# r4dl/StopThePop-Rasterization

Hardware: AMD Instinct MI355X
Metric: fwd+bwd frames/sec at 1920×1080, 1M Gaussians; PSNR vs reference (higher is better)
Workload: dtype f32

## Files before the change

### stopthepop-rasterization_amd/csrc/stp_binning.hip

```cpp
#include <cstdlib>
#include <cstring>
#include <rocprim/rocprim.hpp>

#include "stp_internal.h"
#include "stp_device.h"

namespace stp {

uint32_t higher_msb(uint32_t n)
{
    uint32_t msb = sizeof(n) * 4, step = msb;
    while (step > 1) {
        step /= 2;
        if (n >> msb) msb += step; else msb -= step;
    }
    if (n >> msb) msb++;
    return msb;
}

size_t scan_temp_bytes(size_t P)
{
    size_t bytes = 0;
    (void)rocprim::inclusive_scan(nullptr, bytes, (uint32_t*)nullptr, (uint32_t*)nullptr, P, rocprim::plus<uint32_t>());
    return bytes;
}

#include <rocprim/rocprim_version.hpp>
#if ROCPRIM_VERSION_MAJOR == 4 && ROCPRIM_VERSION_MINOR == 2
#define STP_OWN_ONESWEEP 1
#else
#define STP_OWN_ONESWEEP 0
#warning "stp_binning.hip: the own onesweep driver is written against rocPRIM 4.2; with this rocPRIM the tile-bit sort uses rocprim::radix_sort_pairs (check rocprim::detail::onesweep_* against this version, then extend the #if)"
#endif
namespace {
#if STP_OWN_ONESWEEP
namespace rpd = rocprim::detail;
using OsConfig = rpd::wrapped_radix_sort_onesweep_config<rocprim::default_config, uint64_t, uint32_t>;
constexpr rpd::radix_sort_onesweep_config_params os_params()
{
    rpd::radix_sort_onesweep_config_params p = OsConfig::architecture_config<rpd::target_arch::gfx950>::params;
    p.sort.items_per_thread = 8;
#ifdef STP_OS_SORT_BLOCK
    p.sort.block_size = STP_OS_SORT_BLOCK;
#endif
#ifdef STP_OS_SORT_IPT
    p.sort.items_per_thread = STP_OS_SORT_IPT;
#endif
#ifdef STP_OS_HIST_BLOCK
    p.histogram.block_size = STP_OS_HIST_BLOCK;
#endif
#ifdef STP_OS_HIST_IPT
    p.histogram.items_per_thread = STP_OS_HIST_IPT;
#endif
    return p;
}
constexpr rpd::radix_sort_onesweep_config_params OS = os_params();
constexpr unsigned OS_RADIX = 1u << OS.radix_bits_per_place;
constexpr unsigned OS_HIST_ITEMS = OS.histogram.block_size * OS.histogram.items_per_thread;
constexpr unsigned OS_SORT_ITEMS = OS.sort.block_size * OS.sort.items_per_thread;
constexpr unsigned OS_MAX_PLACES = 4;
using OsBlockId = rpd::block_id_wrapper<unsigned int, true>;

struct OsLayout {
    uint32_t* offsets;
    unsigned int* block_ids;
    rpd::onesweep_lookback_state* lookback;
    uint32_t* offsets_tmp;
    uint64_t* keys_tmp;
    uint32_t* values_tmp;
    size_t zero_bytes, total, lookback_offset;
    uint32_t sort_blocks;
};
OsLayout os_layout(char* base, size_t R)
{
    OsLayout L{};
    auto up = [](size_t v) { return (v + 255) & ~(size_t)255; };
    L.sort_blocks = (uint32_t)((R + OS_SORT_ITEMS - 1) / OS_SORT_ITEMS);
    size_t off = 0;
    L.offsets = reinterpret_cast<uint32_t*>(base + off); off += up(sizeof(uint32_t) * OS_MAX_PLACES * OS_RADIX);
    L.block_ids = reinterpret_cast<unsigned int*>(base + off); off += up(sizeof(unsigned int) * OS_MAX_PLACES);
    L.lookback = reinterpret_cast<rpd::onesweep_lookback_state*>(base + off);
    L.lookback_offset = off;
    off += up(sizeof(rpd::onesweep_lookback_state) * OS_MAX_PLACES * OS_RADIX * (size_t)L.sort_blocks);
    L.zero_bytes = off;
    L.offsets_tmp = reinterpret_cast<uint32_t*>(base + off); off += up(sizeof(uint32_t) * OS_RADIX);
    L.keys_tmp = reinterpret_cast<uint64_t*>(base + off); off += up(sizeof(uint64_t) * R);
    L.values_tmp = reinterpret_cast<uint32_t*>(base + off); off += up(sizeof(uint32_t) * R);
    L.total = off;
    return L;
}

__global__ void __launch_bounds__(OS.histogram.block_size) os_histograms_kernel(const uint64_t* keys, uint32_t* counts, uint32_t size, uint32_t full_blocks, unsigned begin_bit, unsigned end_bit)
{
    rpd::onesweep_histograms<OS.histogram.block_size, OS.histogram.items_per_thread, OS.radix_bits_per_place, false>(
        keys, counts, size, full_blocks, rocprim::identity_decomposer{}, begin_bit, end_bit);
}
__global__ void __launch_bounds__(OS.histogram.block_size) os_scan_histograms_kernel(uint32_t* offsets)
{
    rpd::onesweep_scan_histograms<OS.histogram.block_size, OS.radix_bits_per_place>(offsets);
}
__global__ void __launch_bounds__(OS.sort.block_size) os_iteration_kernel(const uint64_t* keys_in, uint64_t* keys_out, const uint32_t* values_in, uint32_t* values_out, unsigned size,
                                                                         uint32_t* offsets_in, uint32_t* offsets_out, rpd::onesweep_lookback_state* lookback, unsigned bit,
                                                                         unsigned radix_bits, unsigned full_blocks, OsBlockId ordered_bid)
{
    rpd::onesweep_iteration<OS.sort.block_size, OS.sort.items_per_thread, OS.radix_bits_per_place, false, OS.radix_rank_algorithm>(
        keys_in, keys_out, values_in, values_out, size, offsets_in, offsets_out, lookback, rocprim::identity_decomposer{}, bit, radix_bits, full_blocks, ordered_bid);
}

constexpr uint32_t OWN_MIN = 1u << 16, OWN_MAX = 1u << 30;
bool own_onesweep_driver(size_t R)
{
    const bool lib = switches().tile_sort == Switches::TILE_SORT_ROCPRIM;
    const bool always = switches().tile_sort == Switches::TILE_SORT_OWN;
    return !lib && (R >= OWN_MIN || (always && R > 0)) && R < OWN_MAX;
}
#else
struct OsLayout { size_t total; };
OsLayout os_layout(char*, size_t) { return OsLayout{0}; }
bool own_onesweep_driver(size_t) { return false; }
#endif
}

size_t sort_temp_bytes(size_t R)
{
    size_t bytes = 0;
    (void)rocprim::radix_sort_pairs(nullptr, bytes, (uint64_t*)nullptr, (uint64_t*)nullptr, (uint32_t*)nullptr, (uint32_t*)nullptr,
                                    R, 0u, 64u);
    const size_t own = os_layout(nullptr, R).total;
    return bytes > own ? bytes : own;
}

void sort_zero_region(const BinningState& b, size_t R, uint32_t tiles, uint32_t** ptr, size_t* words)
{
    *ptr = nullptr; *words = 0;
    if (!own_onesweep_driver(R)) return;
#if STP_OWN_ONESWEEP
    const OsLayout L = os_layout(b.sort_temp, R);
    const uint32_t bit = higher_msb(tiles);
    const size_t places = (bit + OS.radix_bits_per_place - 1) / OS.radix_bits_per_place;
    const size_t bytes = L.lookback_offset + ((sizeof(rpd::onesweep_lookback_state) * places * OS_RADIX * (size_t)L.sort_blocks + 255) & ~(size_t)255);
    *ptr = reinterpret_cast<uint32_t*>(b.sort_temp);
    *words = (bytes < L.zero_bytes ? bytes : L.zero_bytes) / sizeof(uint32_t);
#else
    (void)b; (void)tiles;
#endif
}

hipError_t launch_scan(const FrameParams& f, const GeometryState& g, hipStream_t st)
{
    size_t bytes = g.scan_temp_bytes;
    return rocprim::inclusive_scan(g.scan_temp, bytes, g.tiles_touched, g.point_offsets, (size_t)f.P, rocprim::plus<uint32_t>(), st);
}

hipError_t launch_sort(const FrameParams& f, const BinningState& b, int R, bool tile_bits_only, bool zeroed, hipStream_t st)
{
    if (R <= 0) return hipSuccess;
    const uint32_t bit = higher_msb((uint32_t)(f.gx * f.gy));
    if (!(tile_bits_only && zeroed && own_onesweep_driver((size_t)R))) {
        size_t bytes = b.sort_temp_bytes;
        return rocprim::radix_sort_pairs(b.sort_temp, bytes, b.keys_unsorted, b.keys, b.point_list_unsorted, b.point_list, (size_t)R,
                                         tile_bits_only ? 32u : 0u, 32u + bit, st);
    }
#if STP_OWN_ONESWEEP
    const OsLayout L = os_layout(b.sort_temp, (size_t)R);
    const unsigned begin_bit = 32u, end_bit = 32u + bit;
    const unsigned places = (bit + OS.radix_bits_per_place - 1) / OS.radix_bits_per_place;
    const uint32_t size = (uint32_t)R;
    {
        const uint32_t blocks = (size + OS_HIST_ITEMS - 1) / OS_HIST_ITEMS, full_blocks = size % OS_HIST_ITEMS == 0 ? blocks : blocks - 1;
        hipLaunchKernelGGL(os_histograms_kernel, dim3(blocks), dim3(OS.histogram.block_size), 0, st, b.keys_unsorted, L.offsets, size, full_blocks, begin_bit, end_bit);
        hipLaunchKernelGGL(os_scan_histograms_kernel, dim3(places), dim3(OS.histogram.block_size), 0, st, L.offsets);
    }
    const uint32_t blocks = L.sort_blocks, full_blocks = size % OS_SORT_ITEMS == 0 ? blocks : blocks - 1;
    bool to_output = (places - 1) % 2 == 0, from_input = true;
    for (unsigned place = 0, pbit = begin_bit; place < places; place++, pbit += OS.radix_bits_per_place) {
        const uint64_t* kin = from_input ? b.keys_unsorted : (to_output ? L.keys_tmp : b.keys);
        const uint32_t* vin = from_input ? b.point_list_unsorted : (to_output ? L.values_tmp : b.point_list);
        uint64_t* kout = to_output ? b.keys : L.keys_tmp;
        uint32_t* vout = to_output ? b.point_list : L.values_tmp;
        const unsigned radix_bits = end_bit - pbit < OS.radix_bits_per_place ? end_bit - pbit : OS.radix_bits_per_place;
        hipLaunchKernelGGL(os_iteration_kernel, dim3(blocks), dim3(OS.sort.block_size), 0, st, kin, kout, vin, vout, size, L.offsets + place * OS_RADIX, L.offsets_tmp,
                           L.lookback + (size_t)place * OS_RADIX * blocks, pbit, radix_bits, full_blocks, OsBlockId::create(L.block_ids + place));
        from_input = false;
        to_output = !to_output;
    }
#endif
    return hipGetLastError();
}

namespace {

constexpr int SCAN_THREADS = 1024;

__global__ void __launch_bounds__(SCAN_THREADS) tile_scan_kernel(int tile0, int T, const uint32_t* __restrict__ counts_, uint2* __restrict__ ranges_,
                                                                 uint32_t* __restrict__ cursor_, uint32_t* __restrict__ total)
{
    const uint32_t* __restrict__ counts = counts_ + tile0;
    uint2* __restrict__ ranges = ranges_ + tile0;
    uint32_t* __restrict__ cursor = cursor_ + tile0;
    __shared__ uint32_t s_part[SCAN_THREADS];
    const int tid = (int)threadIdx.x;
    const int per = (T + SCAN_THREADS - 1) / SCAN_THREADS;
    const int lo = min(tid * per, T), hi = min(lo + per, T);
    uint32_t sum = 0;
    for (int t = lo; t < hi; t++) sum += counts[t];
    s_part[tid] = sum;
    __syncthreads();
    for (int off = 1; off < SCAN_THREADS; off <<= 1) {
        const uint32_t v = tid >= off ? s_part[tid - off] : 0u;
        __syncthreads();
        s_part[tid] += v;
        __syncthreads();
    }
    uint32_t run = s_part[tid] - sum;
    for (int t = lo; t < hi; t++) {
        const uint32_t c = counts[t];
        ranges[t] = c ? make_uint2(run, run + c) : make_uint2(0u, 0u);
        cursor[t] = run;
        run += c;
    }
    if (tid == SCAN_THREADS - 1) total[0] = s_part[tid];
}

__global__ void __launch_bounds__(256) bin_pad_kernel(int R, const uint32_t* __restrict__ total, uint64_t* __restrict__ keys, uint32_t* __restrict__ list)
{
    for (int i = (int)total[0] + (int)threadIdx.x; i < R; i += 256) {
        keys[i] = make_sort_key(INVALID_TILE_ID, FLT_MAX);
        list[i] = 0xFFFFFFFFu;
    }
}

}

hipError_t launch_tile_scan(const FrameParams& f, const ImageState& img, hipStream_t st)
{
    hipLaunchKernelGGL(tile_scan_kernel, dim3(1), dim3(SCAN_THREADS), 0, st, f.gx * f.ty0, f.gx * (f.ty1 - f.ty0), img.tile_counts, img.ranges, img.tile_cursor, img.bin_total);
    return hipGetLastError();
}

hipError_t launch_bin_pad(const BinningState& b, const ImageState& img, int R, hipStream_t st)
{
    if (R <= 0) return hipSuccess;
    hipLaunchKernelGGL(bin_pad_kernel, dim3(1), dim3(256), 0, st, R, img.bin_total, b.keys, b.point_list);
    return hipGetLastError();
}

}
```

### stopthepop-rasterization_amd/csrc/stp_buffers.hip

```cpp
#include "stp_internal.h"
#include "stp_layout_cache.h"

#include <cstring>
#include <mutex>
#include <string>

namespace stp {

GeometryState carve_geometry(char* base, size_t P, bool with_inv, size_t* total, NamedOffset* names, int* n_names, float** sh_stash)
{
    Carver c(base);
    GeometryState g{};
    size_t off;
    int n = 0;
    auto note = [&](const char* nm, size_t o, size_t cnt) { if (names) names[n] = {nm, o, cnt}; n++; };
    g.status = c.take<uint32_t>(64, &off);
    g.depths = c.take<float>(P, &off); note("depths", off, P);
    g.clamped = c.take<uint8_t>(3 * P, &off); note("clamped", off, 3 * P);
    g.internal_radii = c.take<int32_t>(P, &off); note("radii", off, P);
    g.rects2D = c.take<float2>(P, &off); note("rects2D", off, 2 * P);
    g.means2D = c.take<float2>(P, &off); note("means2D", off, 2 * P);
    g.cov3D = c.take<float>(6 * P, &off); note("cov3D", off, 6 * P);
    if (with_inv) { g.cov3D_inv = c.take<float4>(3 * P, &off); note("cov3D_inv", off, 12 * P); }
    if (with_inv) { g.gpack = c.take<float4>(4 * P, &off); note("gpack", off, 16 * P); }
    g.conic_opacity = c.take<float4>(P, &off); note("conic_opacity", off, 4 * P);
    g.rgb = c.take<float>(3 * P, &off); note("rgb", off, 3 * P);
    g.tiles_touched = c.take<uint32_t>(P, &off); note("tiles_touched", off, P);
    g.point_offsets = c.take<uint32_t>(P, &off); note("point_offsets", off, P);
    g.block_sums = c.take<uint32_t>((P + 255) / 256, &off);
    g.block_prefix = c.take<uint32_t>((P + 255) / 256, &off);
    g.scan_temp_bytes = scan_temp_bytes(P);
    g.scan_temp = c.take<char>(g.scan_temp_bytes);
    g.invz = c.take<float>(P, &off); note("invz", off, P);
    {
        const Carver before_stash = c;
        float* const stash = c.take<float>(9 * P, &off); note("sh_stash", off, 9 * P);
        if (sh_stash) *sh_stash = stash;
        else c = before_stash;
    }
    if (total) *total = c.total();
    if (n_names) *n_names = n;
    return g;
}

ImageState carve_image(char* base, int W, int H, int ty0, int ty1, int log_depth, size_t* total, NamedOffset* names, int* n_names)
{
    Carver c(base);
    ImageState s{};
    size_t off;
    int n = 0;
    auto note = [&](const char* nm, size_t o, size_t cnt) { if (names) names[n] = {nm, o, cnt}; n++; };
    const int gx = (W + TILE - 1) / TILE;
    const int py0 = ty0 * TILE < H ? ty0 * TILE : H, py1 = ty1 * TILE < H ? ty1 * TILE : H;
    const size_t N = (size_t)W * (size_t)(py1 > py0 ? py1 - py0 : 0), T = (size_t)gx * (size_t)(ty1 > ty0 ? ty1 - ty0 : 0);
    s.header = c.take<uint32_t>(64, &off); note("header", off, 4);
    s.final_T = c.take<float>(N, &off); note("final_T", off, N);
    s.n_contrib = c.take<uint32_t>(N, &off); note("n_contrib", off, N);
    s.ranges = c.take<uint2>(T, &off); note("ranges", off, 2 * T);
    s.dbg_minmax = c.take<uint32_t>(2, &off); note("dbg_minmax", off, 2);
    s.tile_counts = c.take<uint32_t>(T, &off); note("tile_counts", off, T);
    s.tile_cursor = c.take<uint32_t>(T, &off); note("tile_cursor", off, T);
    s.bin_total = c.take<uint32_t>(2, &off); note("bin_total", off, 2);
    s.tile_flags = c.take<uint32_t>(T, &off); note("tile_flags", off, T);
    const size_t recs_per_tile = 4 * (size_t)blend_log_rows(log_depth) * 64;
    s.log_depth = log_depth;
    if (log_depth > 0) {
        const size_t recs = T * recs_per_tile;
        s.blend_log = c.take<uint32_t>(recs / 2, &off); note("blend_log", off, recs);
    }
    if (total) *total = c.total();
    if (n_names) *n_names = n;
    if (base) {
        const size_t pix0 = (size_t)W * (size_t)py0, tile0 = (size_t)gx * (size_t)ty0;
        s.final_T -= pix0; s.n_contrib -= pix0;
        s.ranges -= tile0; s.tile_counts -= tile0; s.tile_cursor -= tile0; s.tile_flags -= tile0;
        if (s.blend_log) s.blend_log -= tile0 * (recs_per_tile / 2);
    }
    return s;
}

BinningState carve_binning(char* base, size_t R, size_t* total, NamedOffset* names, int* n_names)
{
    Carver c(base);
    BinningState b{};
    size_t off;
    int n = 0;
    auto note = [&](const char* nm, size_t o, size_t cnt) { if (names) names[n] = {nm, o, cnt}; n++; };
    b.header = c.take<uint32_t>(64, &off); note("header", off, 4);
    b.point_list = c.take<uint32_t>(R, &off); note("point_list", off, R);
    b.point_list_unsorted = c.take<uint32_t>(R, &off); note("point_list_unsorted", off, R);
    b.keys = c.take<uint64_t>(R, &off); note("keys", off, R);
    b.keys_unsorted = c.take<uint64_t>(R, &off); note("keys_unsorted", off, R);
    b.sort_temp_bytes = sort_temp_bytes(R);
    b.sort_temp = c.take<char>(b.sort_temp_bytes);
    b.entA = c.take<float4>(R, &off); note("entA", off, 4 * R);
    b.entB = c.take<float4>(R, &off); note("entB", off, 4 * R);
    b.entC = c.take<float4>(R, &off); note("entC", off, 4 * R);
    b.entD = c.take<float4>(R, &off); note("entD", off, 4 * R);
    b.entF = c.take<float4>(R, &off); note("entF", off, 4 * R);
    if (total) *total = c.total();
    if (n_names) *n_names = n;
    return b;
}

void clamp_tile_rows(int height, int& y0, int& y1)
{
    const int gy = (height + TILE - 1) / TILE;
    if (y1 <= 0) { y0 = 0; y1 = gy; return; }
    y0 = y0 < 0 ? 0 : (y0 > gy ? gy : y0);
    y1 = y1 > gy ? gy : y1;
    if (y1 < y0) y1 = y0;
}

static std::mutex g_layout_mutex;
static LayoutCache g_layout, g_log_depth, g_stash;
void remember_layout(const void* binning, uint32_t count, int64_t R) { std::lock_guard<std::mutex> l(g_layout_mutex); g_layout.put(binning, count, R); }
void remember_log_depth(const void* image, uint32_t depth, int64_t R) { std::lock_guard<std::mutex> l(g_layout_mutex); g_log_depth.put(image, depth, R); }
void remember_stash(const void* geometry, bool stash, int64_t R) { std::lock_guard<std::mutex> l(g_layout_mutex); g_stash.put(geometry, stash ? 1u : 0u, R); }
static int read_buffer_header(const uint32_t* dev_header, uint32_t magic, const char* what, uint32_t* value, hipStream_t st, bool have_stream)
{
    uint32_t h[4] = {0, 0, 0, 0};
    if (!have_stream) (void)hipDeviceSynchronize();
    if (hipMemcpyAsync(h, dev_header, sizeof(h), hipMemcpyDeviceToHost, have_stream ? st : nullptr) != hipSuccess ||
        hipStreamSynchronize(have_stream ? st : nullptr) != hipSuccess) { (void)hipGetLastError(); return fail(STP_ERR_HIP, std::string("could not read the header of the ") + what + " buffer"); }
    if (h[0] != magic || h[2] != ~h[1])
        return fail(STP_ERR_INVALID_ARGUMENT, std::string("the ") + what + " buffer does not carry a header of this library: it was not written by stp_forward (or has been overwritten)");
    *value = h[1];
    return 0;
}
int layout_of(const char* binning, uint32_t R, uint32_t* cap, hipStream_t st, bool have_stream)
{
    {
        std::lock_guard<std::mutex> l(g_layout_mutex);
        if (g_layout.get(binning, (int64_t)R, cap) && *cap >= R) return 0;
    }
    if (int rc = read_buffer_header(reinterpret_cast<const uint32_t*>(binning), STP_HEADER_MAGIC_BINNING, "binning", cap, st, have_stream)) return rc;
    if (*cap < R) return fail(STP_ERR_INVALID_ARGUMENT, "the binning buffer was carved for fewer entries than num_rendered");
    remember_layout(binning, *cap, (int64_t)R);
    return 0;
}

int log_depth_of(const char* image, int64_t R, uint32_t* depth, hipStream_t st, bool have_stream)
{
    {
        std::lock_guard<std::mutex> l(g_layout_mutex);
        if (g_log_depth.get(image, R, depth)) return 0;
    }
    if (int rc = read_buffer_header(reinterpret_cast<const uint32_t*>(image), STP_HEADER_MAGIC_IMAGE, "image", depth, st, have_stream)) return rc;
    if (*depth != 0u && (int)*depth != blend_log_clamp_depth((int)*depth)) return fail(STP_ERR_INVALID_ARGUMENT, "the image buffer's header holds an impossible blend-log depth");
    remember_log_depth(image, *depth, R);
    return 0;
}

int stash_of(const char* geometry, int P, int64_t R, bool* stash, hipStream_t st, bool have_stream)
{
    uint32_t v = 0;
    {
        std::lock_guard<std::mutex> l(g_layout_mutex);
        if (g_stash.get(geometry, R, &v)) { *stash = v != 0u; return 0; }
    }
    uint32_t h[4] = {0, 0, 0, 0};
    if (!have_stream) (void)hipDeviceSynchronize();
    if (hipMemcpyAsync(h, reinterpret_cast<const uint32_t*>(geometry) + STP_STASH_WORD, sizeof(h), hipMemcpyDeviceToHost, have_stream ? st : nullptr) != hipSuccess ||
        hipStreamSynchronize(have_stream ? st : nullptr) != hipSuccess) { (void)hipGetLastError(); return fail(STP_ERR_HIP, "could not read the status block of the geometry buffer"); }
    *stash = h[0] == STP_HEADER_MAGIC_STASH && h[1] == (uint32_t)P && h[2] == ~(uint32_t)P;
    remember_stash(geometry, *stash, R);
    return 0;
}

}

using namespace stp;

extern "C" {

size_t stp_geometry_buffer_size(int P, const StpSettings* settings)
{
    size_t total = 0;
    carve_geometry(nullptr, (size_t)P, settings ? requires_depth_along_ray(*settings) : true, &total);
    return total;
}
size_t stp_geometry_buffer_size_stash(int P, const StpSettings* settings)
{
    size_t total = 0;
    float* stash = nullptr;
    carve_geometry(nullptr, (size_t)P, settings ? requires_depth_along_ray(*settings) : true, &total, nullptr, nullptr, &stash);
    return total;
}
size_t stp_binning_buffer_size(int R)
{
    size_t total = 0;
    carve_binning(nullptr, (size_t)(R > 0 ? R : 0), &total);
    return total;
}
size_t stp_image_buffer_size(int width, int height)
{
    size_t total = 0;
    carve_image(nullptr, width, height, 0, (height + TILE - 1) / TILE, 0, &total);
    return total;
}

static size_t blend_log_bytes_of(int width, int height, int tile_y0, int tile_y1, int depth)
{
    clamp_tile_rows(height, tile_y0, tile_y1);
    size_t plain = 0, with_log = 0;
    carve_image(nullptr, width, height, tile_y0, tile_y1, 0, &plain);
    carve_image(nullptr, width, height, tile_y0, tile_y1, depth, &with_log);
    return with_log - plain;
}
size_t stp_blend_log_bytes_rows(int width, int height, int tile_y0, int tile_y1)
{
    return blend_log_bytes_of(width, height, tile_y0, tile_y1, blend_log_default_depth());
}
size_t stp_blend_log_bytes(int width, int height) { return stp_blend_log_bytes_rows(width, height, 0, 0); }
size_t stp_blend_log_bytes_depth(int width, int height, int tile_y0, int tile_y1, int depth)
{
    return blend_log_bytes_of(width, height, tile_y0, tile_y1, depth > 0 ? blend_log_clamp_depth(depth) : blend_log_clamp_depth(1 << 30));
}

static int find_name(const NamedOffset* names, int n, const char* name, size_t* offset, size_t* count)
{
    for (int i = 0; i < n; i++)
        if (std::strcmp(names[i].name, name) == 0) {
            if (offset) *offset = names[i].offset;
            if (count) *count = names[i].count;
            return 0;
        }
    return fail(STP_ERR_INVALID_ARGUMENT, std::string("unknown sub-array name: ") + name);
}
int stp_geometry_layout(int P, const StpSettings* settings, const char* name, size_t* offset, size_t* count)
{
    NamedOffset names[24]; int n = 0;
    carve_geometry(nullptr, (size_t)P, settings ? requires_depth_along_ray(*settings) : true, nullptr, names, &n);
    return find_name(names, n, name, offset, count);
}
int stp_binning_layout(int R, const char* name, size_t* offset, size_t* count)
{
    NamedOffset names[16]; int n = 0;
    carve_binning(nullptr, (size_t)(R > 0 ? R : 0), nullptr, names, &n);
    return find_name(names, n, name, offset, count);
}
void stp_forget_buffer(const void* buffer)
{
    if (!buffer) return;
    std::lock_guard<std::mutex> l(g_layout_mutex);
    g_layout.map.erase(buffer);
    g_log_depth.map.erase(buffer);
    g_stash.map.erase(buffer);
}
int stp_blend_log_depth(const void* image_buffer)
{
    if (!image_buffer) return fail(STP_ERR_INVALID_ARGUMENT, "null image buffer");
    uint32_t d = 0;
    if (int rc = log_depth_of((const char*)image_buffer, -1, &d)) return rc;
    return (int)d;
}
int stp_binning_layout_count(const void* binning_buffer, int R)
{
    if (!binning_buffer) return fail(STP_ERR_INVALID_ARGUMENT, "null binning buffer");
    uint32_t cap = 0;
    if (int rc = layout_of((const char*)binning_buffer, (uint32_t)(R > 0 ? R : 0), &cap)) return rc;
    return (int)cap;
}
static int image_layout_of(int width, int height, int tile_y0, int tile_y1, int depth, const char* name, size_t* offset, size_t* count)
{
    NamedOffset names[16]; int n = 0;
    clamp_tile_rows(height, tile_y0, tile_y1);
    carve_image(nullptr, width, height, tile_y0, tile_y1, depth, nullptr, names, &n);
    return find_name(names, n, name, offset, count);
}
int stp_image_layout_rows(int width, int height, int tile_y0, int tile_y1, const char* name, size_t* offset, size_t* count)
{
    return image_layout_of(width, height, tile_y0, tile_y1, blend_log_default_depth(), name, offset, count);
}
int stp_image_layout(int width, int height, const char* name, size_t* offset, size_t* count)
{
    return stp_image_layout_rows(width, height, 0, 0, name, offset, count);
}
int stp_image_layout_depth(int width, int height, int tile_y0, int tile_y1, int log_depth, const char* name, size_t* offset, size_t* count)
{
    return image_layout_of(width, height, tile_y0, tile_y1, log_depth > 0 ? blend_log_clamp_depth(log_depth) : 0, name, offset, count);
}

}
```

### stopthepop-rasterization_amd/csrc/stp_forward.hip

```cpp
#include "stp_internal.h"

#include <atomic>
#include <cstring>
#include <mutex>
#include <string>

using namespace stp;

namespace {
struct Mailbox { volatile uint32_t* host = nullptr; uint32_t* dev = nullptr; hipEvent_t ev = nullptr; hipEvent_t done = nullptr; int device = 0; uint32_t ticket = 0; };
constexpr int MAILBOX_RING = 8;
struct MailboxRing { Mailbox slot[MAILBOX_RING]; std::atomic<unsigned> next{0}; std::atomic<bool> ready{false};
                     uint32_t* log_need = nullptr;  };
MailboxRing g_mailboxes[MAX_DEVICES];
std::mutex g_mailbox_mutex;
constexpr int GUESS_SLOTS = 16;
struct SizeGuess { std::atomic<uint64_t> key{0}; std::atomic<uint32_t> R{0}; std::atomic<uint32_t> log_need{0}; };
SizeGuess g_guess[MAX_DEVICES][GUESS_SLOTS];
uint64_t guess_key(const FrameParams& f)
{
    uint64_t k = 0x9E3779B97F4A7C15ull;
    for (uint64_t v : {(uint64_t)f.P, (uint64_t)f.W, (uint64_t)f.H, (uint64_t)f.ty0, (uint64_t)f.ty1, (uint64_t)f.s.sort_mode,
                       (uint64_t)(f.s.tile_based_culling * 8 + f.s.rect_bounding * 4 + f.s.tight_opacity_bounding * 2 + (f.s.sort_order == ORDER_PTD_MAX))})
        k = (k ^ v) * 0xBF58476D1CE4E5B9ull, k ^= k >> 29;
    return k | 1ull;
}

struct SideStream { hipStream_t stream = nullptr; std::atomic<bool> ready{false}; };
SideStream g_side[MAX_DEVICES];
SideStream* side_stream(int device)
{
    if (!switches().side_stream || device < 0 || device >= MAX_DEVICES) return nullptr;
    SideStream& s = g_side[device];
    if (!s.ready.load(std::memory_order_acquire)) {
        std::lock_guard<std::mutex> lock(g_mailbox_mutex);
        if (!s.ready.load(std::memory_order_relaxed)) {
            if (hipStreamCreateWithFlags(&s.stream, hipStreamNonBlocking) != hipSuccess) { (void)hipGetLastError(); return nullptr; }
            s.ready.store(true, std::memory_order_release);
        }
    }
    return &s;
}
struct SideJoin {
    hipEvent_t done; hipStream_t st; bool pending;
    hipError_t join() { if (!pending) return hipSuccess; pending = false; return hipStreamWaitEvent(st, done, 0); }
    ~SideJoin() { (void)join(); }
};

inline void cpu_relax()
{
#if defined(__x86_64__) || defined(__i386__)
    __builtin_ia32_pause();
#elif defined(__aarch64__)
    asm volatile("yield" ::: "memory");
#else
    std::atomic_signal_fence(std::memory_order_seq_cst);
#endif
}

constexpr uint32_t RUN_AHEAD_AUTO_MAX = 1u << 18;
std::atomic<int> g_run_ahead{[] { const char* e = std::getenv("STP_RUN_AHEAD"); return (e && (e[0] == '0' || e[0] == '1')) ? e[0] - '0' : 2; }()};

int log_depth_for(const SizeGuess& slot, uint64_t key)
{
    const int fixed = switches().fixed_log_depth;
    if (fixed > 0) return blend_log_clamp_depth((fixed + 1) & ~1);
    const uint32_t need = slot.key.load(std::memory_order_acquire) == key ? slot.log_need.load(std::memory_order_relaxed) : 0u;
    if (need == 0) return blend_log_default_depth();
    return blend_log_clamp_depth((int)((need + need / 8 + 4 + 15) & ~15u));
}

int acquire_mailbox(Mailbox* out)
{
    int device = 0;
    if (hipGetDevice(&device) != hipSuccess || device < 0 || device >= MAX_DEVICES) return fail(STP_ERR_HIP, "hipGetDevice failed");
    MailboxRing& ring = g_mailboxes[device];
    if (!ring.ready.load(std::memory_order_acquire)) {
        std::lock_guard<std::mutex> lock(g_mailbox_mutex);
        if (!ring.ready.load(std::memory_order_relaxed)) {
            for (int i = 0; i < MAILBOX_RING; i++) {
                void* h = nullptr; void* d = nullptr;
                if (hipHostMalloc(&h, 64, hipHostMallocMapped | hipHostMallocCoherent) != hipSuccess || hipHostGetDevicePointer(&d, h, 0) != hipSuccess ||
                    hipEventCreateWithFlags(&ring.slot[i].ev, hipEventDisableTiming) != hipSuccess ||
                    hipEventCreateWithFlags(&ring.slot[i].done, hipEventDisableTiming) != hipSuccess)
                    return fail(STP_ERR_HIP, "cannot create the num_rendered mailbox");
                std::memset(h, 0, 64);
                ring.slot[i].host = static_cast<volatile uint32_t*>(h);
                ring.slot[i].dev = static_cast<uint32_t*>(d);
                ring.slot[i].device = device;
            }
            if (hipMalloc(reinterpret_cast<void**>(&ring.log_need), sizeof(uint32_t) * 64) != hipSuccess || hipMemset(ring.log_need, 0, sizeof(uint32_t) * 64) != hipSuccess)
                return fail(STP_ERR_HIP, "cannot create the blend-log depth words");
            ring.ready.store(true, std::memory_order_release);
        }
    }
    const unsigned seq = ring.next.fetch_add(1u);
    *out = ring.slot[seq % MAILBOX_RING];
    out->ticket = seq + 1u == 0u ? 1u : seq + 1u;
    return 0;
}

struct ForwardCall {
    const hipStream_t st; const int debug;
    FrameParams f;
    GeometryState g{}; ImageState img{}; char* img_ptr = nullptr; char* geom_base = nullptr; float* sh_stash = nullptr;
    Mailbox mb;
    SizeGuess* gslot = nullptr; uint64_t gkey = 0;
    uint32_t* log_need_word = nullptr; uint32_t log_tag = 0; int log_depth = 0; bool with_log = false;
    SideStream* side = nullptr;
    bool colour_started = true;
    char* bin_ptr = nullptr; size_t bin_have = 0;
    uint32_t cap = 0; bool ahead = false, run_ahead = false;
    int* radii; float* const out_color;
    struct Split { const ForwardSplit s; hipStream_t st; bool recorded; ~Split() { if (s.armed && !recorded) (void)hipEventRecord(s.event, st); } } split;
    SideJoin colours;

    ForwardCall(hipStream_t stream, int debug_, const ForwardSplit& split_, int* radii_, float* out_color_)
        : st(stream), debug(debug_), radii(radii_), out_color(out_color_), split{split_, stream, false}, colours{nullptr, stream, false} {}
    int carve_geometry_and_image(stp_alloc_fn geometry_alloc, void* geometry_user, stp_alloc_fn image_alloc, void* image_user, bool with_inv, bool with_stash);
    int launch_up_to_mailbox(); int colour_on_side();
    int request_binning(stp_alloc_fn binning_alloc, void* binning_user);
    int wait_mailbox(); int read_mailbox(int* R_out, bool* wild_out);
    int binning_and_render(const GeometryState& gd, const BinningState& b, int L, uint32_t dup_cap);
};

int ForwardCall::carve_geometry_and_image(stp_alloc_fn geometry_alloc, void* geometry_user, stp_alloc_fn image_alloc, void* image_user, bool with_inv, bool with_stash)
{
    size_t geom_bytes = 0;
    carve_geometry(nullptr, (size_t)f.P, with_inv, &geom_bytes, nullptr, nullptr, with_stash ? &sh_stash : nullptr);
    char* geom_ptr = (char*)geometry_alloc(geometry_user, geom_bytes);
    if (!geom_ptr) return fail(STP_ERR_ALLOC, "geometry allocator returned NULL");
    g = carve_geometry(geom_ptr, (size_t)f.P, with_inv, nullptr, nullptr, nullptr, with_stash ? &sh_stash : nullptr);
    geom_base = geom_ptr;
    if (!radii) radii = g.internal_radii;

    if (int rc = acquire_mailbox(&mb)) return rc;
    colours.done = mb.done;
    gkey = guess_key(f);
    const unsigned gidx = (unsigned)((gkey >> 1) % GUESS_SLOTS);
    gslot = &g_guess[mb.device][gidx];
    log_need_word = g_mailboxes[mb.device].log_need + gidx;
    size_t img_bytes = 0;
    with_log = uses_blend_log(f.s);
    log_depth = with_log ? log_depth_for(*gslot, gkey) : 0;
    f.log_depth = log_depth;
    f.log_need = with_log ? log_need_word : nullptr;
    log_tag = (uint32_t)((gkey >> 40) & 0xFFFFu) | 1u;
    f.log_tag = log_tag;
    carve_image(nullptr, f.W, f.H, f.ty0, f.ty1, log_depth, &img_bytes);
    img_ptr = (char*)image_alloc(image_user, img_bytes);
    if (!img_ptr) return fail(STP_ERR_ALLOC, "image allocator returned NULL");
    img = carve_image(img_ptr, f.W, f.H, f.ty0, f.ty1, log_depth, nullptr);
    return 0;
}

int ForwardCall::launch_up_to_mailbox()
{
    const bool atomic_bin = switches().atomic_bin, two_level_scan = switches().two_level_scan;
    timer_begin_forward();
    timer_mark(0, st);
    STP_TRY(launch_frame_init(g, img, f.gx * f.ty0, f.gx * (f.ty1 - f.ty0), with_log, atomic_bin, st), "frame init launch");
    STP_TRY(launch_preprocess(f, g, radii, atomic_bin ? img.tile_counts : nullptr, st), "preprocess launch");
    STP_DEBUG_SYNC("preprocess");
    if (!two_level_scan) STP_TRY(launch_scan(f, g, st), "inclusive scan");
    STP_DEBUG_SYNC("scan");
    if (atomic_bin) STP_TRY(launch_tile_scan(f, img, st), "tile scan");

    if (two_level_scan) STP_TRY(launch_block_prefix_mailbox(f, g, mb.dev, mb.ticket, log_need_word, st), "workgroup prefixes + mailbox launch");
    else STP_TRY(launch_mailbox(g.point_offsets + (f.P - 1), g.status + 1, mb.dev, mb.ticket, log_need_word, st), "mailbox launch");
    STP_TRY(hipEventRecord(mb.ev, st), "record mailbox event");
    side = side_stream(mb.device);
    colour_started = !(side && switches().colour_late);
    if (side) {
        if (colour_started) { if (int rc = colour_on_side()) return rc; }
    } else STP_TRY(launch_sh_color(f, g, radii, sh_stash, st), "SH colour launch");
    return 0;
}

int ForwardCall::colour_on_side()
{
    STP_TRY(hipStreamWaitEvent(side->stream, mb.ev, 0), "side stream wait");
    STP_TRY(launch_sh_color(f, g, radii, sh_stash, side->stream), "SH colour launch");
    if (hipError_t e = hipEventRecord(mb.done, side->stream); e != hipSuccess) {
        (void)hipStreamSynchronize(side->stream);
        return fail_hip(e, "record colour event");
    }
    colours.pending = true;
    return 0;
}

int ForwardCall::request_binning(stp_alloc_fn binning_alloc, void* binning_user)
{
    const Switches& sw = switches();
    const int run_ahead_mode = g_run_ahead.load(std::memory_order_relaxed);
    run_ahead = run_ahead_mode != 0;
    const uint32_t guess = (sw.speculative_binning && gslot->key.load(std::memory_order_acquire) == gkey) ? gslot->R.load(std::memory_order_relaxed) : 0u;
    ahead = run_ahead && guess > 0 && (run_ahead_mode == 1 || guess < RUN_AHEAD_AUTO_MAX) && sw.two_level_scan && !sw.atomic_bin && !debug;
    cap = guess + guess / 8 + (ahead ? 1024u : 0u);
    if (guess > 0) {
        carve_binning(nullptr, (size_t)cap, &bin_have);
        bin_ptr = (char*)binning_alloc(binning_user, bin_have);
        if (!bin_ptr) return fail(STP_ERR_ALLOC, "binning allocator returned NULL");
    }
    return 0;
}

int ForwardCall::wait_mailbox()
{
    const bool mbx_spin = switches().mailbox_spin;
    if (mbx_spin) {
        for (unsigned it = 1;; it++) {
            if (mb.host[2] == mb.ticket) break;
            if ((it & 255u) == 0u) {
                const hipError_t q = hipEventQuery(mb.ev);
                if (q == hipSuccess) break;
                if (q != hipErrorNotReady) return fail_hip(q, "query (num_rendered)");
                if (it > (1u << 22)) { STP_TRY(hipEventSynchronize(mb.ev), "synchronize (num_rendered)"); break; }
            }
            cpu_relax();
        }
        std::atomic_thread_fence(std::memory_order_acquire);
    } else STP_TRY(hipEventSynchronize(mb.ev), "synchronize (num_rendered)");
    return 0;
}

int ForwardCall::read_mailbox(int* R_out, bool* wild_out)
{
    if (int rc = wait_mailbox()) return rc;
    const uint32_t host_status[2] = {mb.host[0], mb.host[1]};
    const uint32_t word = mb.host[3];
    if (const uint32_t reported = (word >> 16) == log_tag ? (word & 0xFFFFu) : 0u) {
        const uint32_t known = gslot->key.load(std::memory_order_acquire) == gkey ? gslot->log_need.load(std::memory_order_relaxed) : 0u;
        const uint32_t keep = known - known / 32;
        gslot->log_need.store(reported > keep ? reported : keep, std::memory_order_relaxed);
    } else if (gslot->key.load(std::memory_order_acquire) != gkey) gslot->log_need.store(0u, std::memory_order_relaxed);
    if (host_status[1] & 1u) return fail(STP_ERR_PREFILTERED, "Point is filtered although prefiltered is set. This shouldn't happen!");
    *wild_out = (host_status[1] & 2u) != 0;
    *R_out = (int)host_status[0];
    const uint32_t prev = gslot->key.load(std::memory_order_acquire) == gkey ? gslot->R.load(std::memory_order_relaxed) : 0u;
    const uint32_t keep = run_ahead ? prev - prev / 32 : 0u;
    gslot->R.store((uint32_t)*R_out > keep ? (uint32_t)*R_out : keep, std::memory_order_relaxed);
    gslot->key.store(gkey, std::memory_order_release);
    return 0;
}

int ForwardCall::binning_and_render(const GeometryState& gd, const BinningState& b, int L, uint32_t dup_cap)
{
    const bool atomic_bin = switches().atomic_bin, tile_local_sort = switches().tile_local_sort;
    uint32_t* zero_ptr = nullptr; size_t zero_words = 0;
    if (!atomic_bin && tile_local_sort) sort_zero_region(b, (size_t)L, (uint32_t)(f.gx * f.gy), &zero_ptr, &zero_words);
    STP_TRY(launch_duplicate(f, gd, radii, b, atomic_bin ? img.tile_cursor : nullptr, dup_cap, (uint32_t)L, zero_ptr, zero_words, st), "duplicate launch");
    STP_DEBUG_SYNC("duplicate");
    timer_mark(2, st);
    if (!colour_started) {
        STP_TRY(hipEventRecord(mb.ev, st), "record event behind duplicate");
        if (int rc = colour_on_side()) return rc;
        colour_started = true;
    }
    if (atomic_bin) {
        STP_TRY(launch_bin_pad(b, img, L, st), "pad entries");
    } else {
        STP_TRY(launch_sort(f, b, L, tile_local_sort, zero_words != 0, st), "radix sort");
        STP_DEBUG_SYNC("sort");
        STP_TRY(launch_ranges(f, b, img, L, st), "tile ranges");
        STP_DEBUG_SYNC("ranges");
    }
    const bool order_wanted = !atomic_bin && tile_order_used(f);
#ifdef STP_ORDER_MAIN
    const bool order_on_side = false;
#else
    const bool order_on_side = order_wanted && side != nullptr && gather_order_mode() == 0 && f.gx * (f.ty1 - f.ty0) >= 16384;
#endif
    if (order_on_side) {
        STP_TRY(hipEventRecord(mb.ev, st), "record event behind the ranges");
        STP_TRY(hipStreamWaitEvent(side->stream, mb.ev, 0), "side stream wait (ranges)");
        STP_TRY(launch_tile_order(f, img, side->stream), "tile order");
    } else if (order_wanted) STP_TRY(launch_tile_order(f, img, st), "tile order");
    STP_TRY(colours.join(), "join colour stream");
    SideJoin ordering{mb.done, st, false};
    if (order_on_side) {
        if (hipError_t e = hipEventRecord(mb.done, side->stream); e != hipSuccess) {
            (void)hipStreamSynchronize(side->stream);
            return fail_hip(e, "record tile-order event");
        }
        ordering.pending = true;
    }
    if (tile_local_sort) STP_TRY(launch_tile_sort_gather(f, g, b, img, L, atomic_bin, st), "tile sort + entry gather");
    else STP_TRY(launch_gather_entries(f, g, b, L, st), "entry gather");
    STP_DEBUG_SYNC("entry gather");
    STP_TRY(ordering.join(), "join tile order");
    timer_mark(3, st);
    std::string err;
    hipError_t e;
    if (split.s.armed && split.s.row > f.ty0 && split.s.row < f.ty1 && f.s.debug_visualization == 0) {
        FrameParams f1 = f, f2 = f;
        f1.ty1 = split.s.row; f2.ty0 = split.s.row;
        f1.split_launch = f2.split_launch = 1;
        e = launch_render_forward(f1, g, b, img, out_color, st, &err);
        if (e == hipSuccess) { e = hipEventRecord(split.s.event, st); split.recorded = e == hipSuccess; }
        if (e == hipSuccess) e = launch_render_forward(f2, g, b, img, out_color, st, &err);
    } else e = launch_render_forward(f, g, b, img, out_color, st, &err);
    if (e != hipSuccess) {
        if (!err.empty()) return fail(STP_ERR_QUEUE_SIZE, err);
        return fail_hip(e, "render launch");
    }
    STP_DEBUG_SYNC("render");
    STP_TRY(launch_render_debug_finish(f, img, out_color, st), "debug visualisation");
    timer_mark(4, st);
    return 0;
}
}

extern "C" {

void stp_set_run_ahead(int mode) { g_run_ahead.store(mode < 0 ? 0 : (mode > 2 ? 2 : mode), std::memory_order_relaxed); }
int stp_get_run_ahead(void) { return g_run_ahead.load(std::memory_order_relaxed); }
void stp_reset_size_guesses(void)
{
    for (auto& dev : g_guess)
        for (auto& slot : dev) { slot.key.store(0, std::memory_order_release); slot.R.store(0u, std::memory_order_relaxed); slot.log_need.store(0u, std::memory_order_relaxed); }
    int cur = 0;
    if (hipGetDevice(&cur) != hipSuccess) return;
    for (int d = 0; d < MAX_DEVICES; d++)
        if (g_mailboxes[d].ready.load(std::memory_order_acquire) && g_mailboxes[d].log_need && hipSetDevice(d) == hipSuccess) {
            (void)hipDeviceSynchronize();
            (void)hipMemset(g_mailboxes[d].log_need, 0, sizeof(uint32_t) * 64);
        }
    (void)hipSetDevice(cur);
}

int stp_forward(stp_alloc_fn geometry_alloc, void* geometry_user, stp_alloc_fn binning_alloc, void* binning_user,
                stp_alloc_fn image_alloc, void* image_user, int P, int D, int M, const float* background, int width, int height,
                const StpSettings* settings, const float* means3D, const float* shs, const float* colors_precomp,
                const float* opacities, const float* scales, float scale_modifier, const float* rotations,
                const float* cov3D_precomp, const float* viewmatrix, const float* projmatrix, const float* inv_viewprojmatrix,
                const float* cam_pos, float tan_fovx, float tan_fovy, int prefiltered, float* out_color, int* radii, int debug,
                void* stream)
{
    const ForwardRequests req = take_forward_requests();
    ForwardCall c((hipStream_t)stream, debug, req.split, radii, out_color);
    const ForwardBackground& fbg = req.background;
    if (!settings || !geometry_alloc || !binning_alloc || !image_alloc) return fail(STP_ERR_INVALID_ARGUMENT, "null settings or allocator");
    if (P < 0 || width <= 0 || height <= 0) return fail(STP_ERR_INVALID_ARGUMENT, "bad sizes");
    if (P == 0) return 0;
    if (!means3D || !opacities || !background || !viewmatrix || !projmatrix || !inv_viewprojmatrix || !cam_pos || !out_color)
        return fail(STP_ERR_INVALID_ARGUMENT, "null required input");
    if (int rc = check_settings(*settings, false)) return rc;
    if ((fbg.bg_image || fbg.out_alpha) && settings->debug_visualization == STP_DEBUG_DEPTH)
        return fail(STP_ERR_INVALID_ARGUMENT, "alpha output / per-pixel background (stp_set_forward_background) are not available with the debug depth visualisation: its image is not C + T * background");
    if (req.out_invdepth && settings->debug_visualization == STP_DEBUG_DEPTH)
        return fail(STP_ERR_INVALID_ARGUMENT, "the inverse-depth output (stp_set_forward_invdepth) is not available with the debug depth visualisation");
    if (int rc = check_raw_params(req.raw_params, opacities, scales, rotations)) return rc;
    const float* const sh_dc = colors_precomp ? nullptr : req.sh_dc;
    if (sh_dc && M > 1 && !shs) return fail(STP_ERR_INVALID_ARGUMENT, "split SH (stp_set_forward_split_sh): M > 1 needs the rest of the coefficients in shs");
    if (!colors_precomp && !shs && !sh_dc) return fail(STP_ERR_INVALID_ARGUMENT, "neither SHs nor precomputed colours given");
    if (!cov3D_precomp && !(scales && rotations)) return fail(STP_ERR_INVALID_ARGUMENT, "neither scale/rotation nor precomputed covariance given");
    const bool with_inv = requires_depth_along_ray(*settings);
    if (with_inv && !(scales && rotations)) return fail(STP_ERR_NEEDS_SCALE_ROTATION, "sorted modes need scales and rotations");

    FrameParams& f = c.f;
    fill_frame(f, P, D, M, background, width, height, *settings, means3D, shs, colors_precomp, opacities, scales, scale_modifier,
               rotations, cov3D_precomp, viewmatrix, projmatrix, inv_viewprojmatrix, cam_pos, tan_fovx, tan_fovy, prefiltered);
    f.out_invdepth = req.out_invdepth;
    f.sh_dc = sh_dc;
    f.raw_params = req.raw_params;
    f.bg_image = fbg.bg_image; f.out_alpha = fbg.out_alpha;
    const bool with_stash = req.sh_stash && !colors_precomp && (shs || sh_dc) && M > 0;
    if (int rc = c.carve_geometry_and_image(geometry_alloc, geometry_user, image_alloc, image_user, with_inv, with_stash)) return rc;

    const Switches& sw = switches();
    f.fused_gather = sw.fused_gather && sw.tile_local_sort && !sw.atomic_bin && f.s.sort_mode == MODE_HIER && f.s.debug_visualization != STP_DEBUG_DEPTH ? 1 : 0;
    if (!sw.two_level_scan) { c.g.block_sums = nullptr; c.g.block_prefix = nullptr; }

    if (int rc = c.launch_up_to_mailbox()) return rc;
    if (int rc = c.request_binning(binning_alloc, binning_user)) return rc;

    const hipStream_t st = c.st;
    int R = 0;
    bool wild = false;
    GeometryState g_dup = c.g;
    if (c.ahead) {
        f.wild_cov = 0;
        timer_mark(1, st);
        const BinningState b = carve_binning(c.bin_ptr, (size_t)c.cap, nullptr);
        if (int rc = c.binning_and_render(g_dup, b, (int)c.cap, c.cap)) return rc;
        if (int rc = c.read_mailbox(&R, &wild)) return rc;
        if ((uint32_t)R <= c.cap && !wild) {
            remember_stash(c.geom_base, with_stash, R);
            remember_layout(c.bin_ptr, c.cap, R);
            remember_log_depth(c.img_ptr, (uint32_t)c.log_depth, R);
            return R;
        }
        g_dup.block_prefix = nullptr; g_dup.block_sums = nullptr;
        STP_TRY(launch_frame_init(c.g, c.img, f.gx * f.ty0, f.gx * (f.ty1 - f.ty0), c.with_log, sw.atomic_bin, st), "frame init launch");
        STP_TRY(launch_stash_mark(f, c.g, c.sh_stash, st), "stash mark launch");
    } else {
        if (int rc = c.read_mailbox(&R, &wild)) return rc;
        STP_DEBUG_SYNC("SH colour");
        timer_mark(1, st);
    }
    f.wild_cov = wild ? 1 : 0;
    size_t bin_bytes = 0;
    carve_binning(nullptr, (size_t)R, &bin_bytes);
    if (bin_bytes > c.bin_have) {
        c.bin_ptr = (char*)binning_alloc(binning_user, bin_bytes);
        if (!c.bin_ptr) return fail(STP_ERR_ALLOC, "binning allocator returned NULL");
    }
    const BinningState b = carve_binning(c.bin_ptr, (size_t)R, nullptr);
    if (int rc = c.binning_and_render(g_dup, b, R, 0xFFFFFFFFu)) return rc;
    remember_stash(c.geom_base, with_stash, R);
    if (c.bin_ptr) remember_layout(c.bin_ptr, (uint32_t)R, R);
    remember_log_depth(c.img_ptr, (uint32_t)c.log_depth, R);
    return R;
}
}
```

### stopthepop-rasterization_amd/csrc/stp_internal.h

```cpp
#pragma once

#include <hip/hip_runtime.h>
#include <cstdint>
#include <cstddef>
#include <cstdlib>
#include <string>

#include "../../include/stp_raster.h"
#include "stp_switches.h"

namespace stp {

constexpr int TILE = 16;
constexpr size_t ALIGN = 256;
static_assert(ALIGN == 256, "Switches::carve_skew (stp_switches.h) is masked to a multiple of 256");
constexpr int MAX_DEVICES = 32;

enum SortMode { MODE_GLOBAL = 0, MODE_FULL = 1, MODE_KBUFFER = 2, MODE_HIER = 3 };
enum SortOrder { ORDER_Z = 0, ORDER_DISTANCE = 1, ORDER_PTD_CENTER = 2, ORDER_PTD_MAX = 3 };

inline bool uses_blend_log(const StpSettings& s)
{
    return s.record_blend_log != 0 && s.debug_visualization == 0 && (s.sort_mode == MODE_HIER || s.sort_mode == MODE_KBUFFER);
}

inline int subtile_mask_kind(const StpSettings& s)
{
    if (s.sort_mode == MODE_HIER && s.hierarchical_4x4_culling) return 1;
    return s.sort_mode == MODE_KBUFFER ? 2 : 0;
}

inline bool requires_depth_along_ray(const StpSettings& s)
{
    return s.sort_mode != MODE_GLOBAL || s.sort_order == ORDER_PTD_CENTER || s.sort_order == ORDER_PTD_MAX;
}

struct Carver {
    char* base;
    size_t off = 0;
    explicit Carver(char* b) : base(b) {}
    static size_t skew() { return switches().carve_skew; }
    template <typename T> T* take(size_t count, size_t* off_out = nullptr)
    {
        off = (off + ALIGN - 1) & ~(ALIGN - 1);
        if (off) off += skew();
        if (off_out) *off_out = off;
        T* p = base ? reinterpret_cast<T*>(base + off) : nullptr;
        off += count * sizeof(T);
        return p;
    }
    size_t total() const { return ((off + ALIGN - 1) & ~(ALIGN - 1)) + ALIGN; }
};

struct GeometryState {
    uint32_t* status;
    float* depths;
    uint8_t* clamped;
    int32_t* internal_radii;
    float2* rects2D;
    float2* means2D;
    float* cov3D;
    float4* cov3D_inv;
    float4* gpack;
    float4* conic_opacity;
    float* rgb;
    uint32_t* tiles_touched;
    uint32_t* point_offsets;
    uint32_t* block_sums;
    uint32_t* block_prefix;
    char* scan_temp;
    size_t scan_temp_bytes;
    float* invz;
};
constexpr int STP_STASH_WORD = 8;
constexpr uint32_t STP_HEADER_MAGIC_STASH = 0x53505453u;

struct ImageState {
    float* final_T;
    uint32_t* n_contrib;
    uint2* ranges;
    uint32_t* dbg_minmax;
    uint32_t* tile_counts;
    uint32_t* tile_cursor;
    uint32_t* bin_total;
    uint32_t* header;
    uint32_t* tile_flags;
    uint32_t* blend_log;
    int log_depth;
};

struct BinningState {
    uint32_t* header;
    uint32_t* point_list;
    uint32_t* point_list_unsorted;
    uint64_t* keys;
    uint64_t* keys_unsorted;
    char* sort_temp;
    size_t sort_temp_bytes;
    float4* entA;
    float4* entB;
    float4* entC;
    float4* entD;
    float4* entF;
};

constexpr uint32_t STP_HEADER_MAGIC_BINNING = 0x42505453u, STP_HEADER_MAGIC_IMAGE = 0x49505453u;
struct NamedOffset { const char* name; size_t offset; size_t count; };

GeometryState carve_geometry(char* base, size_t P, bool with_inv, size_t* total, NamedOffset* names = nullptr, int* n_names = nullptr, float** sh_stash = nullptr);
ImageState carve_image(char* base, int W, int H, int ty0, int ty1, int log_depth , size_t* total, NamedOffset* names = nullptr, int* n_names = nullptr);
BinningState carve_binning(char* base, size_t R, size_t* total, NamedOffset* names = nullptr, int* n_names = nullptr);
void clamp_tile_rows(int height, int& y0, int& y1);

int fail(int code, const std::string& msg);
int fail_hip(hipError_t e, const char* what);
#define STP_TRY(expr, what) do { hipError_t _e = (expr); if (_e != hipSuccess) return fail_hip(_e, what); } while (0)
#define STP_DEBUG_SYNC(what)  STP_TRY(debug ? hipStreamSynchronize(st) : hipSuccess, what)

void timer_begin_forward();
void timer_begin_backward();
void timer_mark(int i, hipStream_t st);

void remember_layout(const void* binning, uint32_t count, int64_t R);
void remember_stash(const void* geometry, bool stash, int64_t R);
int stash_of(const char* geometry, int P, int64_t R, bool* stash, hipStream_t st, bool have_stream);
void remember_log_depth(const void* image, uint32_t depth, int64_t R);
int layout_of(const char* binning, uint32_t R, uint32_t* cap, hipStream_t st = nullptr, bool have_stream = false);
int log_depth_of(const char* image, int64_t R, uint32_t* depth, hipStream_t st = nullptr, bool have_stream = false);

int blend_log_rows(int depth);
int blend_log_default_depth();
int blend_log_clamp_depth(int d);
size_t scan_temp_bytes(size_t P);
size_t sort_temp_bytes(size_t R);

struct FrameParams {
    int P, D, M, W, H, gx, gy;
    int ty0, ty1;
    float focal_x, focal_y, tan_fovx, tan_fovy, scale_modifier;
    StpSettings s;
    const float* background;
    const float* means3D;
    const float* shs;
    const float* colors_precomp;
    const float* opacities;
    const float* scales;
    const float* rotations;
    const float* cov3D_precomp;
    const float* viewmatrix;
    const float* projmatrix;
    const float* inv_viewprojmatrix;
    const float* cam_pos;
    int prefiltered;
    int log_depth;
    uint32_t* log_need;
    uint32_t log_tag;
    int split_launch = 0;
    int fused_gather = 0;
    const float* bg_image = nullptr;
    float* out_alpha = nullptr;
    float* out_invdepth = nullptr;
    const float* sh_dc = nullptr;
    int raw_params = 0;
    int wild_cov;
};

struct CameraGradRequest {
    float* dL_dview = nullptr;
    float* dL_dproj = nullptr;
    float* dL_dcam = nullptr;
    void* workspace = nullptr;
    size_t workspace_bytes = 0;
};

struct BackwardParams {
    CameraGradRequest cam;
    float* absgrad = nullptr;
    float* blend_stats = nullptr;
    const float* bg_image = nullptr;
    const float* dL_dalpha = nullptr;
    float* dL_dbackground = nullptr;
    const float* invdepth = nullptr;
    const float* dL_dinvdepth = nullptr;
    const float* pixel_colors;
    const float* dL_dpix;
    float* grad_rec;
    int grad_stride;
    int clear_rec;
    int chunk, chunks;
    float* dL_dmean2D;
    float* dL_dopacity;
    float* dL_dcolor;
    float* dL_dmean3D;
    float* dL_dcov3D;
    float* dL_dsh;
    float* dL_dscale;
    float* dL_drot;
    const float* sh_stash = nullptr;
    float* dL_ddc = nullptr;
};

int check_settings(const StpSettings& s, bool backward);
void fill_frame(FrameParams& f, int P, int D, int M, const float* background, int width, int height, const StpSettings& s, const float* means3D,
                const float* shs, const float* colors_precomp, const float* opacities, const float* scales, float scale_modifier, const float* rotations,
                const float* cov3D_precomp, const float* viewmatrix, const float* projmatrix, const float* inv_viewprojmatrix, const float* cam_pos,
                float tan_fovx, float tan_fovy, int prefiltered);

struct ForwardSplit { int row = 0; hipEvent_t event = nullptr; bool armed = false; };
struct ForwardBackground { const float* bg_image = nullptr; float* out_alpha = nullptr; };
struct ForwardRequests { ForwardSplit split; ForwardBackground background; float* out_invdepth = nullptr;  const float* sh_dc = nullptr;  bool sh_stash = false;  int raw_params = 0;  };
ForwardRequests take_forward_requests();
int check_raw_params(int mask, const float* opacities, const float* scales, const float* rotations);

hipError_t launch_preprocess(const FrameParams& f, const GeometryState& g, int* radii, uint32_t* tile_counts, hipStream_t st);
hipError_t launch_frame_init(const GeometryState& g, const ImageState& img, int tile0, int n_tiles, bool with_log, bool tile_counters, hipStream_t st);
hipError_t launch_scan(const FrameParams& f, const GeometryState& g, hipStream_t st);
bool tile_order_enabled();
inline bool tile_order_used(const FrameParams& f) { return tile_order_enabled() && f.gx * (f.ty1 - f.ty0) > 1024; }
bool gather_order_enabled();
int gather_order_mode();
hipError_t launch_tile_order(const FrameParams& f, const ImageState& img, hipStream_t st);
hipError_t launch_sh_color(const FrameParams& f, const GeometryState& g, const int* radii, float* sh_stash, hipStream_t st);
hipError_t launch_stash_mark(const FrameParams& f, const GeometryState& g, float* sh_stash, hipStream_t st);
hipError_t launch_mailbox(const uint32_t* last_offset, const uint32_t* status, uint32_t* mailbox_dev, uint32_t ticket, uint32_t* log_need, hipStream_t st);
hipError_t launch_block_prefix_mailbox(const FrameParams& f, const GeometryState& g, uint32_t* mailbox_dev, uint32_t ticket, uint32_t* log_need, hipStream_t st);
hipError_t launch_duplicate(const FrameParams& f, const GeometryState& g, const int* radii, const BinningState& b, uint32_t* tile_cursor, uint32_t cap, uint32_t header_cap, uint32_t* zero_ptr, size_t zero_words, hipStream_t st);
hipError_t launch_tile_scan(const FrameParams& f, const ImageState& img, hipStream_t st);
hipError_t launch_bin_pad(const BinningState& b, const ImageState& img, int R, hipStream_t st);
hipError_t launch_sort(const FrameParams& f, const BinningState& b, int R, bool tile_bits_only, bool zeroed, hipStream_t st);
void sort_zero_region(const BinningState& b, size_t R, uint32_t tiles, uint32_t** ptr, size_t* words);
hipError_t launch_tile_sort_gather(const FrameParams& f, const GeometryState& g, const BinningState& b, const ImageState& img, int R, bool unordered, hipStream_t st);
hipError_t launch_ranges(const FrameParams& f, const BinningState& b, const ImageState& img, int R, hipStream_t st);
hipError_t launch_gather_entries(const FrameParams& f, const GeometryState& g, const BinningState& b, int R, hipStream_t st);
hipError_t launch_render_forward(const FrameParams& f, const GeometryState& g, const BinningState& b, const ImageState& img,
                                 float* out_color, hipStream_t st, std::string* err);
hipError_t launch_render_debug_finish(const FrameParams& f, const ImageState& img, float* out_color, hipStream_t st);
hipError_t launch_render_backward(const FrameParams& f, const GeometryState& g, const BinningState& b, const ImageState& img,
                                  const BackwardParams& bw, hipStream_t st, std::string* err);
size_t background_grad_partials();
hipError_t launch_background_grad(const FrameParams& f, const ImageState& img, const BackwardParams& bw, float* partials, hipStream_t st);
hipError_t launch_preprocess_backward(const FrameParams& f, const GeometryState& g, const int* radii, const BackwardParams& bw, hipStream_t st);
size_t camera_grad_workspace_bytes(int P);
hipError_t launch_camera_grad_finalize(int P, const CameraGradRequest& cam, hipStream_t st);
hipError_t launch_mark_visible(int P, const float* means3D, const float* viewmatrix, uint8_t* present, hipStream_t st);
int launch_sparse_adam(int n_tensors, const StpAdamTensor* tensors, int N, const void* visible, int visible_kind, float beta1, float beta2,
                       hipStream_t st, hipError_t* err);
int launch_dense_adam(int n_tensors, const StpDenseAdamTensor* tensors, hipStream_t st, hipError_t* err);
int launch_activate_params(int P, const float* scaling, const float* rotation, const float* opacity, float* scales, float* rotations, float* opacities,
                           hipStream_t st, hipError_t* err);
int launch_mcmc_relocation(int n, const float* opacity_old, const float* scale_old, const void* N, int n_kind, int n_max, float* opacity_new,
                           float* scale_new, hipStream_t st, hipError_t* err);
int launch_mcmc_add_noise(int P, float* xyz, const float* scales, const float* rotations, const float* opacities, const float* noise, float noise_scale,
                          float k, float x0, int raw, hipStream_t st, hipError_t* err);
int launch_mip_filter_3d(int P, int C, const float* xyz, const float* views, const float* intrinsics, void* workspace, float* filter_3d, hipStream_t st, hipError_t* err);
int launch_mip_activations_forward(int P, const float* scaling, const float* opacity, const float* filter_3d, float* scales, float* opacities, hipStream_t st,
                                   hipError_t* err);
int launch_mip_activations_backward(int P, const float* scaling, const float* opacity, const float* filter_3d, const float* grad_scales, const float* grad_opacities,
                                    float* grad_scaling, float* grad_opacity, hipStream_t st, hipError_t* err);
size_t mcmc_relocate_scratch_bytes(int P);
int launch_mcmc_sample(int P, const float* opacity, int rule, float min_opacity, int raw, int n_draws, const float* uniforms, void* scratch, uint32_t* weights,
                       int32_t* src, int32_t* count, hipStream_t st, hipError_t* err);
int launch_mcmc_relocate_apply(int P, const int32_t* src, const int32_t* count, int n_tensors, const StpMcmcTensor* tensors, float min_opacity, int raw,
                               int reset_dead_moments, void* scratch, hipStream_t st, hipError_t* err);
int launch_mcmc_add_apply(int P, int n_new, const int32_t* src, const int32_t* count, int n_tensors, const StpMcmcTensor* tensors, float min_opacity, int raw,
                          void* scratch, hipStream_t st, hipError_t* err);
int launch_densify_stats(int P, float* grad_accum, float* denom, float* max_radii2D, const float* grad2d, int grad_stride, const void* visible,
                         int visible_kind, hipStream_t st, hipError_t* err);
int launch_densify_plan(int P, const float* grad_accum, const float* denom, const float* scaling, const float* opacity, const float* max_radii2D,
                        const StpDensifyRule& rule, uint8_t* plan, hipStream_t st, hipError_t* err);
size_t densify_scratch_bytes(int P);
int launch_densify_scan(int P, const uint8_t* plan, void* scratch, uint32_t* offsets, int64_t counts[3], hipStream_t st, hipError_t* err);
int launch_densify_apply(int P, const uint8_t* plan, const uint32_t* offsets, const int64_t counts[3], int n_tensors, const StpDensifyTensor* tensors,
                         const float* noise, float split_shrink, int raw, hipStream_t st, hipError_t* err);
uint32_t photometric_groups(int planes, int H, int W);
int launch_photometric_forward(int planes, int H, int W, const float* image, const float* target, float* out2, float* maps, float* workspace,
                               hipStream_t st, hipError_t* err);
int launch_photometric_backward(int planes, int H, int W, const float* image, const float* target, const float* maps, const float* dL_dout2,
                                float* dL_dimage, hipStream_t st, hipError_t* err);
size_t training_loss_workspace_floats(int planes, int H, int W, int depth_planes);
int launch_training_loss_forward(int planes, int H, int W, const float* image, const float* target, const StpTrainingLoss& x, float* out3, float* maps,
                                 float* workspace, hipStream_t st, hipError_t* err);
int launch_training_loss_backward(int planes, int H, int W, const float* image, const float* target, const StpTrainingLoss& x, const float* maps,
                                  const float* dL_dout3, float* dL_dimage, float* dL_dexposure, float* dL_dinvdepth, float* workspace, hipStream_t st,
                                  hipError_t* err);

size_t knn_scratch_bytes(int P);
int launch_knn_mean_dist2(int P, const float* points, void* scratch, float* mean_dist2, hipStream_t st, hipError_t* err);
size_t spatial_order_scratch_bytes(int P);
int launch_spatial_order(int P, const float* xyz, void* scratch, int32_t* order, uint32_t* codes, hipStream_t st, hipError_t* err);
int launch_gather_rows(int P, int M, const int32_t* index, int n_tensors, const StpGatherTensor* tensors, hipStream_t st, hipError_t* err);

uint32_t higher_msb(uint32_t n);

}
```

### stopthepop-rasterization_amd/csrc/stp_preprocess.hip

```cpp
#include "stp_internal.h"
#include "stp_device.h"
#include "stp_sh_dir.h"
#include "stp_activations.h"

namespace stp {

namespace {

struct PreArgs {
    int P, D, M, W, H, gx, gy, ty0, ty1;
    float focal_x, focal_y, tan_fovx, tan_fovy, scale_modifier;
    int sort_order, rect_bounding, tight_opacity_bounding, tile_based_culling, proper_ewa_scaling, prefiltered;
    int raw;
    const float* means3D;
    const float* scales;
    const float* rotations;
    const float* opacities;
    const float* shs;
    const float* cov3D_precomp;
    const float* colors_precomp;
    const float* view;
    const float* proj;
    const float* cam;
    int* radii;
    GeometryState g;
    uint32_t* tile_counts;
};

__device__ __forceinline__ void sh_to_rgb(int idx, int deg, float3 mean, float3 cam, const float* __restrict__ sh,
                                          uint8_t* __restrict__ clamped, float* __restrict__ rgb)
{
#pragma clang fp contract(off)
    float dx = mean.x - cam.x, dy = mean.y - cam.y, dz = mean.z - cam.z;
    const float len = sqrtf(dx * dx + dy * dy + dz * dz);
    const float x = dx / len, y = dy / len, z = dz / len;
    float res[3];
#pragma unroll
    for (int ch = 0; ch < 3; ch++) res[ch] = kSH_C0 * sh[ch];
    if (deg > 0) {
#pragma unroll
        for (int ch = 0; ch < 3; ch++)
            res[ch] = res[ch] - (kSH_C1 * y) * sh[3 + ch] + (kSH_C1 * z) * sh[6 + ch] - (kSH_C1 * x) * sh[9 + ch];
        if (deg > 1) {
            const float xx = x * x, yy = y * y, zz = z * z, xy = x * y, yz = y * z, xz = x * z;
#pragma unroll
            for (int ch = 0; ch < 3; ch++)
                res[ch] = res[ch] + (kSH_C2[0] * xy) * sh[12 + ch] + (kSH_C2[1] * yz) * sh[15 + ch] +
                          (kSH_C2[2] * (2.0f * zz - xx - yy)) * sh[18 + ch] + (kSH_C2[3] * xz) * sh[21 + ch] +
                          (kSH_C2[4] * (xx - yy)) * sh[24 + ch];
            if (deg > 2) {
#pragma unroll
                for (int ch = 0; ch < 3; ch++)
                    res[ch] = res[ch] + (kSH_C3[0] * y * (3.0f * xx - yy)) * sh[27 + ch] + (kSH_C3[1] * xy * z) * sh[30 + ch] +
                              (kSH_C3[2] * y * (4.0f * zz - xx - yy)) * sh[33 + ch] +
                              (kSH_C3[3] * z * (2.0f * zz - 3.0f * xx - 3.0f * yy)) * sh[36 + ch] +
                              (kSH_C3[4] * x * (4.0f * zz - xx - yy)) * sh[39 + ch] + (kSH_C3[5] * z * (xx - yy)) * sh[42 + ch] +
                              (kSH_C3[6] * x * (xx - 3.0f * yy)) * sh[45 + ch];
            }
        }
    }
#pragma unroll
    for (int ch = 0; ch < 3; ch++) {
        const float r = res[ch] + 0.5f;
        clamped[3 * (size_t)idx + ch] = (r < 0.0f) ? 1 : 0;
        rgb[3 * (size_t)idx + ch] = fmaxf(r, 0.0f);
    }
}

constexpr int COOP_TILES = 64;

__device__ __forceinline__ int wave_lane() { return (int)__builtin_amdgcn_mbcnt_hi(~0u, __builtin_amdgcn_mbcnt_lo(~0u, 0u)); }
__device__ __forceinline__ int lanes_below(unsigned long long m) { return (int)__builtin_amdgcn_mbcnt_hi((unsigned int)(m >> 32), __builtin_amdgcn_mbcnt_lo((unsigned int)m, 0u)); }
__device__ __forceinline__ float bcast_f(float v, int src) { return __int_as_float(__builtin_amdgcn_readlane(__float_as_int(v), src)); }
__device__ __forceinline__ int bcast_i(int v, int src) { return __builtin_amdgcn_readlane(v, src); }

struct PreStageA {
    float3 mean, pv, sc;
    float4 q;
    float c3[6];
    float4 co;
    float thr, radius;
    float2 mean2D, rect_dims;
    int fx0, fy0, fx1, fy1, y0, y1;
};

__device__ __forceinline__ bool preprocess_stage_a(const PreArgs& a, int idx, PreStageA& o)
{
#pragma clang fp contract(off)
    const float3 mean = make_float3(a.means3D[3 * (size_t)idx], a.means3D[3 * (size_t)idx + 1], a.means3D[3 * (size_t)idx + 2]);
    float opacity = a.opacities[idx];
    float3 sc_in = make_float3(0.0f, 0.0f, 0.0f);
    float4 q_in = make_float4(0.0f, 0.0f, 0.0f, 0.0f);
    float c3_in[6] = {0.0f, 0.0f, 0.0f, 0.0f, 0.0f, 0.0f};
    if (a.cov3D_precomp != nullptr) {
#pragma unroll
        for (int k = 0; k < 6; k++) c3_in[k] = a.cov3D_precomp[6 * (size_t)idx + k];
    }
    if (a.scales != nullptr && a.rotations != nullptr) {
        sc_in = make_float3(a.scales[3 * (size_t)idx], a.scales[3 * (size_t)idx + 1], a.scales[3 * (size_t)idx + 2]);
        q_in = reinterpret_cast<const float4*>(a.rotations)[idx];
    }
    if (a.raw != 0) {
        if (a.raw & RAW_OPACITY) opacity = activate_opacity(opacity);
        if (a.scales != nullptr && a.rotations != nullptr) {
            if (a.raw & RAW_SCALE) sc_in = make_float3(activate_scale(sc_in.x), activate_scale(sc_in.y), activate_scale(sc_in.z));
            if (a.raw & RAW_ROTATION) q_in = activate_rotation(q_in, nullptr);
        }
    }
    const float* __restrict__ view = a.view;
    float3 pv;
    pv.x = view[0] * mean.x + view[4] * mean.y + view[8] * mean.z + view[12] * 1.0f;
    pv.y = view[1] * mean.x + view[5] * mean.y + view[9] * mean.z + view[13] * 1.0f;
    pv.z = view[2] * mean.x + view[6] * mean.y + view[10] * mean.z + view[14] * 1.0f;
    if (pv.z <= 0.2f) {
        if (a.prefiltered) atomicOr(&a.g.status[1], 1u);
        return false;
    }

    float c3[6];
    if (a.cov3D_precomp != nullptr) {
#pragma unroll
        for (int k = 0; k < 6; k++) c3[k] = c3_in[k];
    } else {
        const float3 sc = sc_in;
        const float4 q = q_in;
        const Mat3 S = mat_diag(a.scale_modifier * sc.x, a.scale_modifier * sc.y, a.scale_modifier * sc.z);
        const Mat3 Mm = mat_mul(S, quat_to_mat(q));
        const Mat3 Sig = mat_mul(mat_transpose(Mm), Mm);
        c3[0] = Sig.m[0][0]; c3[1] = Sig.m[0][1]; c3[2] = Sig.m[0][2]; c3[3] = Sig.m[1][1]; c3[4] = Sig.m[1][2]; c3[5] = Sig.m[2][2];
#pragma unroll
        for (int k = 0; k < 6; k++) a.g.cov3D[6 * (size_t)idx + k] = c3[k];
    }

    float3 t = pv;
    const float limx = 1.3f * a.tan_fovx, limy = 1.3f * a.tan_fovy;
    const float txtz = t.x / t.z, tytz = t.y / t.z;
    t.x = fminf(limx, fmaxf(-limx, txtz)) * t.z;
    t.y = fminf(limy, fmaxf(-limy, tytz)) * t.z;
    Mat3 J;
    J.m[0][0] = a.focal_x / t.z; J.m[0][1] = 0.0f;              J.m[0][2] = -(a.focal_x * t.x) / (t.z * t.z);
    J.m[1][0] = 0.0f;              J.m[1][1] = a.focal_y / t.z; J.m[1][2] = -(a.focal_y * t.y) / (t.z * t.z);
    J.m[2][0] = 0.0f;              J.m[2][1] = 0.0f;              J.m[2][2] = 0.0f;
    Mat3 Wv;
#pragma unroll
    for (int i = 0; i < 3; i++)
#pragma unroll
        for (int j = 0; j < 3; j++) Wv.m[i][j] = view[4 * i + j];
    const Mat3 T = mat_mul(mat_transpose(Wv), J);
    Mat3 Vrk;
    Vrk.m[0][0] = c3[0]; Vrk.m[0][1] = c3[1]; Vrk.m[0][2] = c3[2];
    Vrk.m[1][0] = c3[1]; Vrk.m[1][1] = c3[3]; Vrk.m[1][2] = c3[4];
    Vrk.m[2][0] = c3[2]; Vrk.m[2][1] = c3[4]; Vrk.m[2][2] = c3[5];
    const Mat3 cov = mat_mul(mat_mul(mat_transpose(T), mat_transpose(Vrk)), T);

    float c2x = cov.m[0][0], c2y = cov.m[0][1], c2z = cov.m[1][1];
    c2x += 0.3f; c2z += 0.3f;
    const float det = c2x * c2z - c2y * c2y;
    float conv_scale = 1.0f;
    if (a.proper_ewa_scaling) {
        const float det_orig = cov.m[0][0] * cov.m[1][1] - cov.m[0][1] * cov.m[0][1];
        conv_scale = sqrtf(fmaxf(0.000025f, det_orig / det));
    }
    if (det == 0.0f) return false;
    const float det_inv = 1.f / det;
    const float4 co = make_float4(c2z * det_inv, -c2y * det_inv, c2x * det_inv, opacity * conv_scale);
    if (co.w < ALPHA_THRESHOLD) return false;

    const float thr = log_rounded(co.w / ALPHA_THRESHOLD);
    const float extent = a.tight_opacity_bounding ? (float)fmin(3.33, (double)sqrtf(2.0f * thr)) : 3.33f;
    const float mid = 0.5f * (c2x + c2z);
    const float lambda = mid + sqrtf(fmaxf(0.01f, mid * mid - det));
    const float radius = extent * sqrtf(lambda);
    if (radius <= 0.0f) return false;

    const float* __restrict__ proj = a.proj;
    float ph[4];
#pragma unroll
    for (int j = 0; j < 4; j++) ph[j] = (proj[j] * mean.x + proj[4 + j] * mean.y) + (proj[8 + j] * mean.z + proj[12 + j] * 1.0f);
    const float p_w = 1.0f / (ph[3] + 0.0000001f);
    const float2 mean2D = make_float2(ndc_to_pix(ph[0] * p_w, a.W), ndc_to_pix(ph[1] * p_w, a.H));

    const float ext_x = fminf(a.rect_bounding ? (extent * sqrtf(c2x)) : radius, radius);
    const float ext_y = fminf(a.rect_bounding ? (extent * sqrtf(c2z)) : radius, radius);
    const float2 rect_dims = make_float2(ext_x, ext_y);
    int fx0, fy0, fx1, fy1;
    get_rect(mean2D, rect_dims, a.gx, a.gy, 0, a.gy, fx0, fy0, fx1, fy1);
    if ((fx1 - fx0) * (fy1 - fy0) == 0) return false;
    o.sc = sc_in; o.q = q_in;
    o.mean = mean; o.pv = pv; o.co = co; o.thr = thr; o.radius = radius; o.mean2D = mean2D; o.rect_dims = rect_dims;
#pragma unroll
    for (int k = 0; k < 6; k++) o.c3[k] = c3[k];
    o.fx0 = fx0; o.fy0 = fy0; o.fx1 = fx1; o.fy1 = fy1;
    o.y0 = min(max(fy0, a.ty0), fy1); o.y1 = max(min(fy1, a.ty1), o.y0);
    return true;
}

__global__ void __launch_bounds__(256) preprocess_kernel(const PreArgs a)
{
#pragma clang fp contract(off)
    const int idx = blockIdx.x * blockDim.x + threadIdx.x;
    PreStageA o{};
    bool alive = false;
    if (idx < a.P) {
        a.radii[idx] = 0;
        a.g.tiles_touched[idx] = 0;
        alive = preprocess_stage_a(a, idx, o);
    }

    const int x0 = o.fx0, x1 = o.fx1, y0 = o.y0, y1 = o.y1;
    int tile_count = (x1 - x0) * (y1 - y0);
    int full_count = 1;
    const bool tbc = a.tile_based_culling != 0;
    const int rect_tiles = (o.fx1 - o.fx0) * (o.fy1 - o.fy0);
    const bool coop = alive && tbc && a.tile_counts == nullptr && rect_tiles > COOP_TILES;
    if (alive && tbc && !coop) {
        tile_count = 0;
        full_count = 0;
        for (int y = o.fy0; y < o.fy1; y++)
            for (int x = o.fx0; x < o.fx1; x++) {
                const float2 tmin = make_float2((float)(x * TILE), (float)(y * TILE));
                const float2 tmax = make_float2((float)((x + 1) * TILE - 1), (float)((y + 1) * TILE - 1));
                float2 mp;
                const float f = max_contrib_power_rect(o.co, o.mean2D, tmin, tmax, (float)(TILE - 1), (float)(TILE - 1), mp);
                const int hit = (f <= o.thr) ? 1 : 0;
                full_count += hit;
                const int mine = (y >= y0 && y < y1) ? hit : 0;
                tile_count += mine;
                if (mine && a.tile_counts) atomicAdd(&a.tile_counts[y * a.gx + x], 1u);
            }
    } else if (alive && !tbc && a.tile_counts) {
        for (int y = y0; y < y1; y++)
            for (int x = x0; x < x1; x++) atomicAdd(&a.tile_counts[y * a.gx + x], 1u);
    }
    {
        const int lane = wave_lane();
        unsigned long long todo = __ballot(coop);
        while (todo) {
            const int src = (int)__builtin_ctzll(todo);
            todo &= todo - 1ull;
            const float4 co = make_float4(bcast_f(o.co.x, src), bcast_f(o.co.y, src), bcast_f(o.co.z, src), bcast_f(o.co.w, src));
            const float2 m2 = make_float2(bcast_f(o.mean2D.x, src), bcast_f(o.mean2D.y, src));
            const float thr = bcast_f(o.thr, src);
            const int sx0 = bcast_i(o.fx0, src), sy0 = bcast_i(o.fy0, src), sx1 = bcast_i(o.fx1, src), sy1 = bcast_i(o.fy1, src);
            const int wy0 = bcast_i(o.y0, src), wy1 = bcast_i(o.y1, src);
            const int w = sx1 - sx0, n = w * (sy1 - sy0);
            int full = 0, mine = 0;
            for (int t0 = 0; t0 < n; t0 += 64) {
                const int t = t0 + lane;
                const int ty = t / w, y = sy0 + ty, x = sx0 + (t - ty * w);
                bool hit = false;
                if (t < n) {
                    const float2 tmin = make_float2((float)(x * TILE), (float)(y * TILE));
                    const float2 tmax = make_float2((float)((x + 1) * TILE - 1), (float)((y + 1) * TILE - 1));
                    float2 mp;
                    hit = max_contrib_power_rect(co, m2, tmin, tmax, (float)(TILE - 1), (float)(TILE - 1), mp) <= thr;
                }
                full += (int)__popcll(__ballot(hit));
                mine += (int)__popcll(__ballot(hit && y >= wy0 && y < wy1));
            }
            if (lane == src) { full_count = full; tile_count = mine; }
        }
    }
    uint32_t my_entries = 0u;
    if (alive && full_count != 0) {
        my_entries = (uint32_t)tile_count;

    const float3 mean = o.mean, pv = o.pv;
    const float4 co = o.co;
    const float2 mean2D = o.mean2D, rect_dims = o.rect_dims;
    const float radius = o.radius;
    const float3 cam = make_float3(a.cam[0], a.cam[1], a.cam[2]);

    if (a.g.cov3D_inv != nullptr) {
        const float3 sc = o.sc;
        const float4 q = o.q;
        const Mat3 S = mat_diag(1.f / (a.scale_modifier * fmaxf(1e-3f, sc.x)), 1.f / (a.scale_modifier * fmaxf(1e-3f, sc.y)),
                                1.f / (a.scale_modifier * fmaxf(1e-3f, sc.z)));
        const Mat3 Mm = mat_mul(S, quat_to_mat(q));
        const Mat3 inv = mat_mul(mat_transpose(Mm), Mm);
        const float dx = cam.x - mean.x, dy = cam.y - mean.y, dz = cam.z - mean.z;
        const float ux = (-inv.m[0][0]) * dx + (-inv.m[1][0]) * dy + (-inv.m[2][0]) * dz;
        const float uy = (-inv.m[0][1]) * dx + (-inv.m[1][1]) * dy + (-inv.m[2][1]) * dz;
        const float uz = (-inv.m[0][2]) * dx + (-inv.m[1][2]) * dy + (-inv.m[2][2]) * dz;
        const bool tame = fabsf(inv.m[0][0]) < 1.0e36f && fabsf(inv.m[0][1]) < 1.0e36f && fabsf(inv.m[0][2]) < 1.0e36f &&
                          fabsf(inv.m[1][1]) < 1.0e36f && fabsf(inv.m[1][2]) < 1.0e36f && fabsf(inv.m[2][2]) < 1.0e36f;
        if (!tame) atomicOr(&a.g.status[1], 2u);
        a.g.cov3D_inv[3 * (size_t)idx + 0] = make_float4(inv.m[0][0], inv.m[0][1], inv.m[0][2], 0.0f);
        a.g.cov3D_inv[3 * (size_t)idx + 1] = make_float4(inv.m[1][1], inv.m[1][2], inv.m[2][2], 0.0f);
        a.g.cov3D_inv[3 * (size_t)idx + 2] = make_float4(ux, uy, uz, 0.0f);
    }

    float depth;
    if (a.sort_order == ORDER_Z) depth = pv.z;
    else {
        const float dx = cam.x - mean.x, dy = cam.y - mean.y, dz = cam.z - mean.z;
        depth = sqrtf(dx * dx + dy * dy + dz * dz);
    }
    a.g.depths[idx] = depth;
    a.radii[idx] = (int)ceilf(radius);
    a.g.rects2D[idx] = rect_dims;
    a.g.means2D[idx] = mean2D;
    a.g.conic_opacity[idx] = co;
    a.g.tiles_touched[idx] = (uint32_t)tile_count;
    if (a.g.invz != nullptr) a.g.invz[idx] = 1.0f / pv.z;
    if (a.g.gpack != nullptr) {
        const float4 s0 = a.g.cov3D_inv[3 * (size_t)idx + 0], s1 = a.g.cov3D_inv[3 * (size_t)idx + 1], s2 = a.g.cov3D_inv[3 * (size_t)idx + 2];
        float4* const gp = a.g.gpack + 4 * (size_t)idx;
        gp[0] = make_float4(s0.x, s0.y, s0.z, s1.x);
        gp[1] = make_float4(s1.y, s1.z, s2.x, s2.y);
        gp[2] = make_float4(s2.z, mean2D.x, mean2D.y, 0.0f);
        gp[3] = co;
    }
    }

    if (a.g.block_sums != nullptr) {
        __shared__ uint32_t s_wave_total[4];
        const int lane = wave_lane(), wave = (int)(threadIdx.x >> 6);
        uint32_t v = my_entries;
#pragma unroll
        for (int d = 1; d < 64; d <<= 1) {
            const uint32_t t = (uint32_t)__shfl_up((int)v, d);
            if (lane >= d) v += t;
        }
        if (lane == 63) s_wave_total[wave] = v;
        __syncthreads();
        for (int k = 0; k < wave; k++) v += s_wave_total[k];
        if (idx < a.P) a.g.point_offsets[idx] = v;
        if (threadIdx.x == 255) a.g.block_sums[blockIdx.x] = v;
    }
}

struct ShArgs {
    int P, D, M;
    const float* means3D;
    const float* shs;
    const float* cam;
    const int* radii;
    uint8_t* clamped;
    float* rgb;
    const float* dc;
    float* stash;
    uint32_t* mark;
};

#ifndef STP_SH_BLOCK
#define STP_SH_BLOCK 256
#endif
constexpr int SH_BLOCK = STP_SH_BLOCK;

template <bool SPLIT, bool STASH>
__global__ void __launch_bounds__(SH_BLOCK) sh_color_kernel(const ShArgs a)
{
    extern __shared__ float s_rows[];
    const int tid = (int)threadIdx.x;
    const int base = (int)blockIdx.x * SH_BLOCK;
    const int idx = base + tid;
    const int rows = min(SH_BLOCK, a.P - base);
    const int row_len = 3 * a.M, row_stride = row_len + 1;
    const float* __restrict__ src = a.shs + (size_t)base * (SPLIT ? row_len - 3 : row_len);
    const float* __restrict__ src_dc = SPLIT ? a.dc + (size_t)base * 3 : nullptr;
    const int total = rows * row_len;
    const bool vec = SPLIT ? aligned16(a.dc, row_len > 3 ? a.shs : nullptr) : true;
    const bool fast = row_len == 48 && rows == SH_BLOCK && vec;
    float4 v48[12];
    if constexpr (SPLIT) {
        static_assert(!SPLIT || SH_BLOCK == 256, "split48_* are written for 256 rows");
        if (fast) split48_load(src_dc, src, tid, v48);
    } else {
        if (fast) stage_rows_load<SH_BLOCK, 48>(src, tid, v48);
    }
    const int ic = min(idx, a.P - 1);
    const int radius_ic = a.radii[ic];
    const float3 mean = make_float3(a.means3D[3 * (size_t)ic], a.means3D[3 * (size_t)ic + 1], a.means3D[3 * (size_t)ic + 2]);
    const int my_radius = idx < a.P ? radius_ic : 0;
    if constexpr (SPLIT) {
        if (fast) {
            split48_store(s_rows, tid, v48);
        } else {
            stage_span_in<SH_BLOCK>(src_dc, s_rows, tid, rows, 3, 0, row_stride, vec);
            stage_span_in<SH_BLOCK>(src, s_rows, tid, rows, row_len - 3, 3, row_stride, vec);
        }
    } else if (fast) {
        stage_rows_store<SH_BLOCK, 48>(s_rows, tid, v48);
    } else if ((row_len & 3) == 0) {
        for (int f = 4 * tid; f < total; f += 4 * SH_BLOCK) {
            const float4 v = *reinterpret_cast<const float4*>(src + f);
            const int r = f / row_len, j = f - r * row_len;
            float* d = s_rows + r * row_stride + j;
            d[0] = v.x; d[1] = v.y; d[2] = v.z; d[3] = v.w;
        }
    } else {
        for (int f = tid; f < total; f += SH_BLOCK) {
            const int r = f / row_len, j = f - r * row_len;
            s_rows[r * row_stride + j] = src[f];
        }
    }
    __syncthreads();
    if (my_radius > 0) {
        const float3 cam = make_float3(a.cam[0], a.cam[1], a.cam[2]);
        sh_to_rgb(idx, a.D, mean, cam, s_rows + tid * row_stride, a.clamped, a.rgb);
        if constexpr (STASH) {
            const float* __restrict__ sh_row = s_rows + tid * row_stride;
            float x, y, z;
            sh_unit_dir(make_float3(mean.x - cam.x, mean.y - cam.y, mean.z - cam.z), x, y, z);
            const int D = a.D;
#pragma unroll
            for (int ch = 0; ch < 3; ch++) {
                float sh[16], dx, dy, dz;
#pragma unroll
                for (int k = 1; k < 16; k++) sh[k] = (k < a.M && k < (D + 1) * (D + 1)) ? sh_row[3 * k + ch] : 0.0f;
                sh_dir_derivative(D, x, y, z, sh, dx, dy, dz);
                a.stash[(size_t)(3 * ch + 0) * a.P + idx] = dx; a.stash[(size_t)(3 * ch + 1) * a.P + idx] = dy; a.stash[(size_t)(3 * ch + 2) * a.P + idx] = dz;
            }
        }
    }
    if constexpr (STASH) {
        if (idx == 0) { a.mark[0] = STP_HEADER_MAGIC_STASH; a.mark[1] = (uint32_t)a.P; a.mark[2] = ~(uint32_t)a.P; }
    }
}

__global__ void stash_mark_kernel(uint32_t* mark, uint32_t P) { mark[0] = STP_HEADER_MAGIC_STASH; mark[1] = P; mark[2] = ~P; }

struct DupArgs {
    int P, W, H, gx, gy, ty0, ty1;
    int sort_order, tile_based_culling;
    const float* inv_vp;
    const float* cam;
    const int* radii;
    GeometryState g;
    uint64_t* keys;
    uint32_t* values;
    uint32_t* tile_cursor;
    uint32_t cap;
    int n_gauss_blocks;
    int n_pad_blocks;
    uint32_t* header;
    uint32_t header_cap;
    uint32_t* zero_ptr;
    uint32_t zero_words;
};
constexpr int DUP_PAD_BLOCKS = 128, DUP_ZERO_BLOCKS = 32;

struct DupGaussian { float2 xy; float4 co; float thr; float3 p0, p1, p2; float global_depth; };
__device__ __forceinline__ bool duplicate_tile(const DupArgs& a, const DupGaussian& g, float3 cam, bool tbc, bool eval_max, bool per_tile_depth,
                                               int x, int y, uint64_t& key)
{
#pragma clang fp contract(off)
    const float2 tmin = make_float2((float)(x * TILE), (float)(y * TILE));
    const float2 tmax = make_float2((float)((x + 1) * TILE - 1), (float)((y + 1) * TILE - 1));
    float2 max_pos = make_float2(0, 0);
    float max_fac = 0.0f;
    if (eval_max) max_fac = max_contrib_power_rect(g.co, g.xy, tmin, tmax, (float)(TILE - 1), (float)(TILE - 1), max_pos);
    float depth = g.global_depth;
    if (per_tile_depth) {
        const float2 center = make_float2((tmin.x + tmax.x) * 0.5f, (tmin.y + tmax.y) * 0.5f);
        const float2 target = (a.sort_order == ORDER_PTD_MAX) ? max_pos : center;
        const float3 dir = view_ray(a.inv_vp, cam, target.x, target.y, a.W, a.H);
        depth = fmaxf(0.0f, depth_along_ray(g.p0, g.p1, g.p2, dir) + 8.0f);
    }
    key = make_sort_key((uint32_t)(y * a.gx + x), depth);
    return !tbc || max_fac <= g.thr;
}

__global__ void __launch_bounds__(256) duplicate_kernel(const DupArgs a)
{
#pragma clang fp contract(off)
    if (blockIdx.x == 0 && threadIdx.x == 0 && a.header) { a.header[0] = STP_HEADER_MAGIC_BINNING; a.header[1] = a.header_cap; a.header[2] = ~a.header_cap; a.header[3] = 0u; }
    if ((int)blockIdx.x >= a.n_gauss_blocks + a.n_pad_blocks) {
        uint4* const z = reinterpret_cast<uint4*>(a.zero_ptr);
        for (uint32_t i = ((uint32_t)blockIdx.x - (uint32_t)(a.n_gauss_blocks + a.n_pad_blocks)) * 256u + threadIdx.x; i < a.zero_words / 4u; i += (uint32_t)DUP_ZERO_BLOCKS * 256u)
            z[i] = make_uint4(0u, 0u, 0u, 0u);
        return;
    }
    if ((int)blockIdx.x >= a.n_gauss_blocks) {
        const int nb = a.n_gauss_blocks;
        const uint32_t total = a.g.block_prefix[nb - 1] + a.g.block_sums[nb - 1];
        for (uint64_t i = (uint64_t)total + ((uint32_t)blockIdx.x - (uint32_t)nb) * 256u + threadIdx.x; i < (uint64_t)a.cap; i += (uint64_t)DUP_PAD_BLOCKS * 256u) {
            a.values[i] = 0xFFFFFFFFu;
            a.keys[i] = make_sort_key(INVALID_TILE_ID, FLT_MAX);
        }
        return;
    }
    const int idx = blockIdx.x * blockDim.x + threadIdx.x;
    const bool valid = idx < a.P && a.radii[idx] > 0;
    const bool tbc = a.tile_based_culling != 0;
    const bool per_tile_depth = a.sort_order == ORDER_PTD_CENTER || a.sort_order == ORDER_PTD_MAX;
    const bool eval_max = tbc || a.sort_order == ORDER_PTD_MAX;
    uint32_t off = 0, off_to = 0;
    int x0 = 0, y0 = 0, x1 = 0, y1 = 0;
    DupGaussian g{};
    float3 cam = make_float3(0, 0, 0);
    if (per_tile_depth) cam = make_float3(a.cam[0], a.cam[1], a.cam[2]);
    if (a.g.block_prefix != nullptr) {
        if (idx < a.P) {
            const uint32_t base = a.g.block_prefix[blockIdx.x];
            off = base + (threadIdx.x == 0 ? 0u : a.g.point_offsets[idx - 1]);
            off_to = base + a.g.point_offsets[idx];
        }
        __syncthreads();
        if (idx < a.P) a.g.point_offsets[idx] = off_to;
    } else if (valid) {
        off = (idx == 0) ? 0u : a.g.point_offsets[idx - 1];
        off_to = a.g.point_offsets[idx];
    }
    if (valid) {
        g.xy = a.g.means2D[idx];
        const float2 ext = a.g.rects2D[idx];
        get_rect(g.xy, ext, a.gx, a.gy, a.ty0, a.ty1, x0, y0, x1, y1);
        if (eval_max) {
            g.co = a.g.conic_opacity[idx];
            g.thr = log_rounded(g.co.w / ALPHA_THRESHOLD);
        }
        if (per_tile_depth) {
            g.p0 = f4_xyz(a.g.cov3D_inv[3 * (size_t)idx + 0]);
            g.p1 = f4_xyz(a.g.cov3D_inv[3 * (size_t)idx + 1]);
            g.p2 = f4_xyz(a.g.cov3D_inv[3 * (size_t)idx + 2]);
        }
        g.global_depth = a.g.depths[idx];
    }
    const bool coop = valid && a.tile_cursor == nullptr && (x1 - x0) * (y1 - y0) > COOP_TILES;
    if (valid && !coop) {
        for (int y = y0; y < y1; y++)
            for (int x = x0; x < x1; x++) {
                uint64_t key;
                if (duplicate_tile(a, g, cam, tbc, eval_max, per_tile_depth, x, y, key)) {
                    if (a.tile_cursor) {
                        const uint32_t slot = atomicAdd(&a.tile_cursor[(uint32_t)(key >> 32)], 1u);
                        a.values[slot] = (uint32_t)idx;
                        a.keys[slot] = key;
                    } else if (off < off_to && off < a.cap) {
                        a.values[off] = (uint32_t)idx;
                        a.keys[off] = key;
                    }
                    off++;
                }
            }
        if (!a.tile_cursor)
            for (; off < off_to && off < a.cap; off++) {
                a.values[off] = 0xFFFFFFFFu;
                a.keys[off] = make_sort_key(INVALID_TILE_ID, FLT_MAX);
            }
    }
    const int lane = wave_lane();
    unsigned long long todo = __ballot(coop);
    while (todo) {
        const int src = (int)__builtin_ctzll(todo);
        todo &= todo - 1ull;
        DupGaussian s;
        s.xy = make_float2(bcast_f(g.xy.x, src), bcast_f(g.xy.y, src));
        s.co = make_float4(bcast_f(g.co.x, src), bcast_f(g.co.y, src), bcast_f(g.co.z, src), bcast_f(g.co.w, src));
        s.thr = bcast_f(g.thr, src);
        s.p0 = make_float3(bcast_f(g.p0.x, src), bcast_f(g.p0.y, src), bcast_f(g.p0.z, src));
        s.p1 = make_float3(bcast_f(g.p1.x, src), bcast_f(g.p1.y, src), bcast_f(g.p1.z, src));
        s.p2 = make_float3(bcast_f(g.p2.x, src), bcast_f(g.p2.y, src), bcast_f(g.p2.z, src));
        s.global_depth = bcast_f(g.global_depth, src);
        const int sx0 = bcast_i(x0, src), sy0 = bcast_i(y0, src), sx1 = bcast_i(x1, src), sy1 = bcast_i(y1, src);
        const uint32_t s_to = (uint32_t)bcast_i((int)off_to, src), s_idx = (uint32_t)bcast_i(idx, src);
        uint32_t base = (uint32_t)bcast_i((int)off, src);
        const int w = sx1 - sx0, n = w * (sy1 - sy0);
        for (int t0 = 0; t0 < n; t0 += 64) {
            const int t = t0 + lane;
            const int ty = t / w;
            uint64_t key = 0;
            const bool wr = t < n && duplicate_tile(a, s, cam, tbc, eval_max, per_tile_depth, sx0 + (t - ty * w), sy0 + ty, key);
            const unsigned long long wm = __ballot(wr);
            const uint32_t slot = base + (uint32_t)lanes_below(wm);
            if (wr && slot < s_to && slot < a.cap) { a.values[slot] = s_idx; a.keys[slot] = key; }
            base += (uint32_t)__popcll(wm);
        }
        for (uint32_t p = base + (uint32_t)lane; p < s_to && p < a.cap; p += 64u) {
            a.values[p] = 0xFFFFFFFFu;
            a.keys[p] = make_sort_key(INVALID_TILE_ID, FLT_MAX);
        }
    }
}

__global__ void __launch_bounds__(256) tile_ranges_kernel(int L, const uint64_t* __restrict__ keys, uint2* __restrict__ ranges, uint32_t T)
{
    const int idx = blockIdx.x * blockDim.x + threadIdx.x;
    if (idx >= L) return;
    const uint32_t cur = (uint32_t)(keys[idx] >> 32);
    const bool valid = cur != INVALID_TILE_ID && cur < T;
    if (idx == 0) {
        if (valid) ranges[cur].x = 0;
    } else {
        const uint32_t prev = (uint32_t)(keys[idx - 1] >> 32);
        if (cur != prev) {
            if (prev < T) ranges[prev].y = (uint32_t)idx;
            if (valid) ranges[cur].x = (uint32_t)idx;
        }
    }
    if (idx == L - 1 && valid) ranges[cur].y = (uint32_t)L;
}

__global__ void __launch_bounds__(1024) tile_order_kernel(int tile0, int T, const uint2* __restrict__ ranges_, uint32_t* __restrict__ order, uint32_t* __restrict__ gather_order)
{
    __shared__ uint32_t s_hist[256];
    __shared__ uint32_t s_hx[8 * 256];
    const uint2* __restrict__ ranges = ranges_ + tile0;
    const int tid = (int)threadIdx.x;
    auto klass = [](uint32_t len) { return 255u - (len < 2048u ? (len >> 4) : min(127u, (len - 2048u) >> 7) + 128u); };
    const int xq = T >> 3, xr = T & 7;
    auto xcd_of = [&](int t) { const int cut = xr * (xq + 1); return t < cut ? t / (xq + 1) : xr + (xq ? (t - cut) / xq : 0); };
    if (tid < 256) s_hist[tid] = 0u;
    for (int i = tid; i < 8 * 256; i += 1024) s_hx[i] = 0u;
    __syncthreads();
    for (int t = tid; t < T; t += 1024) {
        const uint32_t c = klass(ranges[t].y - ranges[t].x);
        atomicAdd(&s_hist[c], 1u);
        if (gather_order) atomicAdd(&s_hx[xcd_of(t) * 256 + c], 1u);
    }
    __syncthreads();
    const int wv = tid >> 6, ln = tid & 63;
    if (wv < (gather_order ? 9 : 1)) {
        uint32_t* const h = wv == 0 ? s_hist : s_hx + (wv - 1) * 256;
        uint32_t c[4], sum = 0;
        for (int k = 0; k < 4; k++) { c[k] = h[4 * ln + k]; sum += c[k]; }
        uint32_t inc = sum;
        for (int o = 1; o < 64; o <<= 1) { const uint32_t v = __shfl_up(inc, o); if (ln >= o) inc += v; }
        uint32_t run = inc - sum;
        for (int k = 0; k < 4; k++) { h[4 * ln + k] = run; run += c[k]; }
    }
    __syncthreads();
    for (int t = tid; t < T; t += 1024) {
        const uint32_t c = klass(ranges[t].y - ranges[t].x);
        order[atomicAdd(&s_hist[c], 1u)] = (uint32_t)t;
        if (gather_order) { const int x = xcd_of(t); gather_order[8u * atomicAdd(&s_hx[x * 256 + c], 1u) + (uint32_t)x] = (uint32_t)t; }
    }
}

__global__ void __launch_bounds__(256) mark_visible_kernel(int P, const float* __restrict__ means3D, const float* __restrict__ view, uint8_t* __restrict__ present)
{
#pragma clang fp contract(off)
    const int idx = blockIdx.x * blockDim.x + threadIdx.x;
    if (idx >= P) return;
    const float z = view[2] * means3D[3 * (size_t)idx] + view[6] * means3D[3 * (size_t)idx + 1] + view[10] * means3D[3 * (size_t)idx + 2] + view[14] * 1.0f;
    present[idx] = z > 0.2f ? 1 : 0;
}

}

hipError_t launch_preprocess(const FrameParams& f, const GeometryState& g, int* radii, uint32_t* tile_counts, hipStream_t st)
{
    PreArgs a;
    a.P = f.P; a.D = f.D; a.M = f.M; a.W = f.W; a.H = f.H; a.gx = f.gx; a.gy = f.gy; a.ty0 = f.ty0; a.ty1 = f.ty1;
    a.focal_x = f.focal_x; a.focal_y = f.focal_y; a.tan_fovx = f.tan_fovx; a.tan_fovy = f.tan_fovy; a.scale_modifier = f.scale_modifier;
    a.sort_order = f.s.sort_order; a.rect_bounding = f.s.rect_bounding; a.tight_opacity_bounding = f.s.tight_opacity_bounding;
    a.tile_based_culling = f.s.tile_based_culling; a.proper_ewa_scaling = f.s.proper_ewa_scaling; a.prefiltered = f.prefiltered;
    a.raw = f.raw_params;
    a.means3D = f.means3D; a.scales = f.scales; a.rotations = f.rotations; a.opacities = f.opacities; a.shs = f.shs;
    a.cov3D_precomp = f.cov3D_precomp; a.colors_precomp = f.colors_precomp; a.view = f.viewmatrix; a.proj = f.projmatrix; a.cam = f.cam_pos;
    a.radii = radii; a.g = g; a.tile_counts = tile_counts;
    if (f.out_invdepth == nullptr) a.g.invz = nullptr;
    hipLaunchKernelGGL(preprocess_kernel, dim3((f.P + 255) / 256), dim3(256), 0, st, a);
    return hipGetLastError();
}

hipError_t launch_duplicate(const FrameParams& f, const GeometryState& g, const int* radii, const BinningState& b, uint32_t* tile_cursor, uint32_t cap, uint32_t header_cap,
                            uint32_t* zero_ptr, size_t zero_words, hipStream_t st)
{
    DupArgs a;
    a.P = f.P; a.W = f.W; a.H = f.H; a.gx = f.gx; a.gy = f.gy; a.ty0 = f.ty0; a.ty1 = f.ty1;
    a.sort_order = f.s.sort_order; a.tile_based_culling = f.s.tile_based_culling;
    a.inv_vp = f.inv_viewprojmatrix; a.cam = f.cam_pos; a.radii = radii; a.g = g;
    a.tile_cursor = tile_cursor;
    a.keys = tile_cursor ? b.keys : b.keys_unsorted; a.values = tile_cursor ? b.point_list : b.point_list_unsorted;
    const bool capped = cap != 0xFFFFFFFFu && g.block_prefix != nullptr && tile_cursor == nullptr;
    a.cap = capped ? cap : 0xFFFFFFFFu;
    a.n_gauss_blocks = (f.P + 255) / 256;
    a.n_pad_blocks = capped ? DUP_PAD_BLOCKS : 0;
    a.zero_ptr = zero_ptr; a.zero_words = (uint32_t)zero_words;
    a.header = b.header; a.header_cap = header_cap;
    hipLaunchKernelGGL(duplicate_kernel, dim3(a.n_gauss_blocks + a.n_pad_blocks + (zero_words ? DUP_ZERO_BLOCKS : 0)), dim3(256), 0, st, a);
    return hipGetLastError();
}

hipError_t launch_sh_color(const FrameParams& f, const GeometryState& g, const int* radii, float* sh_stash, hipStream_t st)
{
    const bool split = f.sh_dc != nullptr;
    if (f.colors_precomp != nullptr || (f.shs == nullptr && !split) || f.M <= 0) return hipSuccess;
    ShArgs a;
    a.P = f.P; a.D = f.D; a.M = f.M; a.means3D = f.means3D; a.shs = f.shs; a.cam = f.cam_pos; a.radii = radii; a.clamped = g.clamped; a.rgb = g.rgb;
    a.dc = f.sh_dc;
    const bool stash = sh_stash != nullptr;
    a.stash = sh_stash; a.mark = g.status + STP_STASH_WORD;
    using Kernel = void (*)(const ShArgs);
    static const Kernel kernels[4] = {sh_color_kernel<false, false>, sh_color_kernel<true, false>, sh_color_kernel<false, true>, sh_color_kernel<true, true>};
    const Kernel kernel = kernels[(stash ? 2 : 0) + (split ? 1 : 0)];
    const size_t lds = (size_t)SH_BLOCK * (3 * a.M + 1) * sizeof(float);
    if (lds > 64 * 1024) {
        hipError_t e = hipFuncSetAttribute(reinterpret_cast<const void*>(kernel), hipFuncAttributeMaxDynamicSharedMemorySize, (int)lds);
        if (e != hipSuccess) return e;
    }
    hipLaunchKernelGGL(kernel, dim3((f.P + SH_BLOCK - 1) / SH_BLOCK), dim3(SH_BLOCK), lds, st, a);
    return hipGetLastError();
}

hipError_t launch_stash_mark(const FrameParams& f, const GeometryState& g, float* sh_stash, hipStream_t st)
{
    if (sh_stash == nullptr) return hipSuccess;
    hipLaunchKernelGGL(stash_mark_kernel, dim3(1), dim3(1), 0, st, g.status + STP_STASH_WORD, (uint32_t)f.P);
    return hipGetLastError();
}

__global__ void mailbox_kernel(const uint32_t* __restrict__ last_offset, const uint32_t* __restrict__ status, volatile uint32_t* mailbox, uint32_t ticket,
                               uint32_t* log_need)
{
    mailbox[0] = *last_offset;
    mailbox[1] = *status;
    mailbox[3] = log_need ? atomicExch(log_need, 0u) : 0u;
    __threadfence_system();
    mailbox[2] = ticket;
    __threadfence_system();
}

__global__ void __launch_bounds__(1024) block_prefix_mailbox_kernel(const uint32_t* __restrict__ block_sums, uint32_t* __restrict__ block_prefix, int n_blocks,
                                                                     const uint32_t* __restrict__ status, volatile uint32_t* mailbox, uint32_t ticket,
                                                                     uint32_t* log_need)
{
    __shared__ uint32_t s_wave_total[16];
    const int tid = (int)threadIdx.x, lane = tid & 63, wave = tid >> 6;
    const int per = (n_blocks + 1023) / 1024, i0 = min(tid * per, n_blocks), i1 = min(i0 + per, n_blocks);
    uint32_t mine = 0u;
    for (int i = i0; i < i1; i++) mine += block_sums[i];
    uint32_t v = mine;
#pragma unroll
    for (int d = 1; d < 64; d <<= 1) {
        const uint32_t t = (uint32_t)__shfl_up((int)v, d);
        if (lane >= d) v += t;
    }
    if (lane == 63) s_wave_total[wave] = v;
    __syncthreads();
    for (int k = 0; k < wave; k++) v += s_wave_total[k];
    uint32_t run = v - mine;
    for (int i = i0; i < i1; i++) { block_prefix[i] = run; run += block_sums[i]; }
    if (tid == 1023) {
        mailbox[0] = v;
        mailbox[1] = status[1];
        mailbox[3] = log_need ? atomicExch(log_need, 0u) : 0u;
        __threadfence_system();
        mailbox[2] = ticket;
        __threadfence_system();
    }
}

hipError_t launch_block_prefix_mailbox(const FrameParams& f, const GeometryState& g, uint32_t* mailbox_dev, uint32_t ticket, uint32_t* log_need, hipStream_t st)
{
    hipLaunchKernelGGL(block_prefix_mailbox_kernel, dim3(1), dim3(1024), 0, st, g.block_sums, g.block_prefix, (f.P + 255) / 256, g.status, mailbox_dev, ticket, log_need);
    return hipGetLastError();
}

hipError_t launch_mailbox(const uint32_t* last_offset, const uint32_t* status, uint32_t* mailbox_dev, uint32_t ticket, uint32_t* log_need, hipStream_t st)
{
    hipLaunchKernelGGL(mailbox_kernel, dim3(1), dim3(1), 0, st, last_offset, status, mailbox_dev, ticket, log_need);
    return hipGetLastError();
}

__global__ void __launch_bounds__(256) frame_init_kernel(uint32_t* __restrict__ status, uint2* __restrict__ ranges, uint32_t* __restrict__ tile_flags,
                                                          uint32_t flag_value, uint32_t* __restrict__ tile_counts, int tile0, int T,
                                                          uint32_t* __restrict__ header, uint32_t log_depth)
{
    const int i = blockIdx.x * blockDim.x + threadIdx.x;
    if (i < 64) status[i] = 0u;
    if (i == 0) { header[0] = STP_HEADER_MAGIC_IMAGE; header[1] = log_depth; header[2] = ~log_depth; header[3] = 0u; }
    if (i < T) {
        ranges[tile0 + i] = make_uint2(0u, 0u);
        tile_flags[tile0 + i] = flag_value;
        if (tile_counts) tile_counts[tile0 + i] = 0u;
    }
}

hipError_t launch_frame_init(const GeometryState& g, const ImageState& img, int tile0, int T, bool with_log, bool tile_counters, hipStream_t st)
{
    const int n = T > 64 ? T : 64;
    hipLaunchKernelGGL(frame_init_kernel, dim3((n + 255) / 256), dim3(256), 0, st, g.status, img.ranges, img.tile_flags, with_log ? 0u : 0xFFFFFFFFu,
                       tile_counters ? img.tile_counts : nullptr, tile0, T, img.header, (uint32_t)(with_log ? img.log_depth : 0));
    return hipGetLastError();
}

hipError_t launch_ranges(const FrameParams& f, const BinningState& b, const ImageState& img, int R, hipStream_t st)
{
    const size_t T = (size_t)f.gx * f.gy;
    hipError_t e = hipSuccess;
    if (R > 0) {
        hipLaunchKernelGGL(tile_ranges_kernel, dim3((R + 255) / 256), dim3(256), 0, st, R, b.keys, img.ranges, (uint32_t)T);
        e = hipGetLastError();
    }
    return e;
}

bool tile_order_enabled() { return switches().tile_order; }
bool gather_order_enabled() { return gather_order_mode() != 0; }
int gather_order_mode() { return switches().gather_order; }
hipError_t launch_tile_order(const FrameParams& f, const ImageState& img, hipStream_t st)
{
    const int T = f.gx * (f.ty1 - f.ty0);
    if (T <= 0) return hipSuccess;
    hipLaunchKernelGGL(tile_order_kernel, dim3(1), dim3(1024), 0, st, f.gx * f.ty0, T, img.ranges, img.tile_cursor + f.gx * f.ty0,
                       gather_order_enabled() ? img.tile_counts + f.gx * f.ty0 : nullptr);
    return hipGetLastError();
}

__global__ void __launch_bounds__(256) gather_entries_kernel(int R, const uint32_t* __restrict__ point_list, const uint64_t* __restrict__ keys,
                                                             const float4* __restrict__ gpack, const float* __restrict__ features,
                                                             float4* __restrict__ entA, float4* __restrict__ entB, float4* __restrict__ entC,
                                                             float4* __restrict__ entD, float4* __restrict__ entF, int mask_kind, int gx, uint32_t T)
{
    const int i = blockIdx.x * blockDim.x + threadIdx.x;
    if (i >= R) return;
    const int id = (int)point_list[i];
    if (id < 0) return;
    const float4* __restrict__ gp = gpack + 4 * (size_t)id;
    const float4 pa = gp[0], pb = gp[1], pc = gp[2], pd = gp[3];
    entA[i] = pa;
    entB[i] = pb;
    entC[i] = make_float4(pc.x, pc.y, pc.z, __int_as_float(id));
    entD[i] = pd;
    float spare = 0.0f;
    const uint32_t tile = (uint32_t)(keys[i] >> 32);
    if (mask_kind && tile < T) spare = __uint_as_float(subtile_mask(mask_kind, pd, make_float2(pc.y, pc.z), (int)(tile % (uint32_t)gx), (int)(tile / (uint32_t)gx)));
    entF[i] = make_float4(features[3 * (size_t)id], features[3 * (size_t)id + 1], features[3 * (size_t)id + 2], spare);
}

hipError_t launch_gather_entries(const FrameParams& f, const GeometryState& g, const BinningState& b, int R, hipStream_t st)
{
    if (R <= 0 || (f.s.sort_mode != MODE_HIER && f.s.sort_mode != MODE_KBUFFER)) return hipSuccess;
    const float* features = f.colors_precomp ? f.colors_precomp : g.rgb;
    hipLaunchKernelGGL(gather_entries_kernel, dim3((R + 255) / 256), dim3(256), 0, st, R, b.point_list, b.keys, g.gpack, features, b.entA, b.entB, b.entC,
                       b.entD, b.entF, subtile_mask_kind(f.s), f.gx, (uint32_t)(f.gx * f.gy));
    return hipGetLastError();
}

hipError_t launch_mark_visible(int P, const float* means3D, const float* viewmatrix, uint8_t* present, hipStream_t st)
{
    hipLaunchKernelGGL(mark_visible_kernel, dim3((P + 255) / 256), dim3(256), 0, st, P, means3D, viewmatrix, present);
    return hipGetLastError();
}

}
```

### stopthepop-rasterization_amd/csrc/stp_switches.h

```cpp
#pragma once
#include <cstddef>
#include <cstdlib>
#include <cstring>

namespace stp {

struct Switches {
    bool tile_local_sort;
    bool atomic_bin;
    bool fused_gather;
    bool two_level_scan;
    bool colour_late;
    bool speculative_binning;
    bool mailbox_spin;
    bool side_stream;
    int fixed_log_depth;
    size_t carve_skew;
    bool tile_order;
    int gather_order;
    enum TileSort { TILE_SORT_AUTO, TILE_SORT_ROCPRIM, TILE_SORT_OWN } tile_sort;
    enum KBuffer { KBUFFER_RING, KBUFFER_TILE, KBUFFER_WAVE } kbuffer;
};

inline const Switches& switches()
{
    static const Switches table = [] {
        const auto is = [](const char* name, const char* value) { const char* e = std::getenv(name); return e && std::strcmp(e, value) == 0; };
        const auto starts_with_0 = [](const char* name) { const char* e = std::getenv(name); return e && e[0] == '0'; };
        const auto number = [](const char* name) { const char* e = std::getenv(name); return e ? std::atoi(e) : 0; };
        Switches s{};
        s.tile_local_sort = !is("STP_SORT", "radix");
        s.atomic_bin = is("STP_SORT", "counters");
        s.fused_gather = !starts_with_0("STP_FUSED_GATHER");
        s.two_level_scan = !is("STP_SCAN", "rocprim");
        s.colour_late = !starts_with_0("STP_COLOUR_LATE");
        s.speculative_binning = !is("STP_BINNING", "exact");
        s.mailbox_spin = !is("STP_MAILBOX", "event");
        s.side_stream = !is("STP_SIDE_STREAM", "0");
        s.fixed_log_depth = number("STP_LOG_DEPTH");
        const char* skew = std::getenv("STP_CARVE_SKEW");
        s.carve_skew = skew ? ((size_t)std::strtoull(skew, nullptr, 0) & ~(size_t)255) : (size_t)0;
        s.tile_order = !starts_with_0("STP_TILE_ORDER");
        s.gather_order = number("STP_GATHER_ORDER");
        s.tile_sort = is("STP_TILE_SORT", "rocprim") ? Switches::TILE_SORT_ROCPRIM : is("STP_TILE_SORT", "own") ? Switches::TILE_SORT_OWN : Switches::TILE_SORT_AUTO;
        s.kbuffer = is("STP_KBUFFER", "tile") ? Switches::KBUFFER_TILE : is("STP_KBUFFER", "wave") ? Switches::KBUFFER_WAVE : Switches::KBUFFER_RING;
        return s;
    }();
    return table;
}

}
```

### stopthepop-rasterization_amd/diff_gaussian_rasterization/_C.py

```python
from __future__ import annotations

import ctypes
import os
from typing import Tuple

import torch

_HERE = os.path.dirname(os.path.abspath(__file__))
_LIB_NAME = "libstp_raster.so"
_lib = None
_host = None


GRAD_RECORD_FLOATS = 16


class StpSettings(ctypes.Structure):
    _fields_ = [(n, ctypes.c_int32) for n in (
        "sort_mode", "sort_order", "queue_tile_4x4", "queue_tile_2x2", "queue_per_pixel",
        "rect_bounding", "tight_opacity_bounding", "tile_based_culling", "hierarchical_4x4_culling",
        "load_balancing", "proper_ewa_scaling", "tile_y0", "tile_y1", "record_blend_log", "debug_visualization")]


_lib_override = None

_OPTIONAL_SYMBOLS = {
    "stp_camera_grad_workspace_bytes": ([ctypes.c_int], ctypes.c_size_t, "camera gradients"),
    "stp_set_backward_camera_grads": ([ctypes.c_void_p] * 4 + [ctypes.c_size_t], None, "camera gradients"),
    "stp_set_backward_absgrad": ([ctypes.c_void_p], None, "absgrad"),
    "stp_set_backward_blend_stats": ([ctypes.c_void_p], None, "blend statistics"),
    "stp_set_forward_background": ([ctypes.c_void_p] * 2, None, "the alpha output and per-pixel background"),
    "stp_set_backward_background": ([ctypes.c_void_p] * 3, None, "the alpha output and per-pixel background"),
    "stp_set_forward_invdepth": ([ctypes.c_void_p], None, "the inverse-depth output"),
    "stp_set_backward_invdepth": ([ctypes.c_void_p] * 2, None, "the inverse-depth output"),
    "stp_set_forward_split_sh": ([ctypes.c_void_p], None, "split SH inputs"),
    "stp_set_backward_split_sh": ([ctypes.c_void_p] * 2, None, "split SH inputs"),
    "stp_set_forward_sh_stash": ([ctypes.c_int], None, "the SH stash"),
    "stp_set_forward_raw_params": ([ctypes.c_int], None, "raw parameter inputs"),
    "stp_set_backward_raw_params": ([ctypes.c_int], None, "raw parameter inputs"),
    "stp_activate_params": ([ctypes.c_int] + [ctypes.c_void_p] * 7, ctypes.c_int, "raw parameter inputs"),
    "stp_geometry_buffer_size_stash": ([ctypes.c_int, ctypes.POINTER(StpSettings)], ctypes.c_size_t, "the SH stash"),
    "stp_sparse_adam": ([ctypes.c_int, ctypes.c_void_p, ctypes.c_int, ctypes.c_void_p, ctypes.c_int, ctypes.c_float, ctypes.c_float, ctypes.c_void_p],
                        ctypes.c_int, "the sparse Adam step"),
    "stp_dense_adam": ([ctypes.c_int, ctypes.c_void_p, ctypes.c_void_p], ctypes.c_int, "the dense Adam step"),
    "stp_mcmc_relocation": ([ctypes.c_int] + [ctypes.c_void_p] * 3 + [ctypes.c_int] * 2 + [ctypes.c_void_p] * 3, ctypes.c_int, "the 3DGS-MCMC kernels"),
    "stp_mcmc_add_noise": ([ctypes.c_int] + [ctypes.c_void_p] * 5 + [ctypes.c_float] * 3 + [ctypes.c_int, ctypes.c_void_p], ctypes.c_int, "the 3DGS-MCMC kernels"),
    "stp_mcmc_relocate_scratch_bytes": ([ctypes.c_int], ctypes.c_size_t, "the 3DGS-MCMC relocation kernels"),
    "stp_mcmc_sample": ([ctypes.c_int, ctypes.c_void_p, ctypes.c_int, ctypes.c_float, ctypes.c_int, ctypes.c_int] + [ctypes.c_void_p] * 2 + [ctypes.c_size_t] + [ctypes.c_void_p] * 4,
                        ctypes.c_int, "the 3DGS-MCMC relocation kernels"),
    "stp_mcmc_relocate_apply": ([ctypes.c_int] + [ctypes.c_void_p] * 2 + [ctypes.c_int, ctypes.c_void_p, ctypes.c_float, ctypes.c_int, ctypes.c_int, ctypes.c_void_p, ctypes.c_size_t,
                                 ctypes.c_void_p], ctypes.c_int, "the 3DGS-MCMC relocation kernels"),
    "stp_mcmc_add_apply": ([ctypes.c_int] * 2 + [ctypes.c_void_p] * 2 + [ctypes.c_int, ctypes.c_void_p, ctypes.c_float, ctypes.c_int, ctypes.c_void_p, ctypes.c_size_t, ctypes.c_void_p],
                           ctypes.c_int, "the 3DGS-MCMC relocation kernels"),
    "stp_mip_filter_3d": ([ctypes.c_int] * 2 + [ctypes.c_void_p] * 6, ctypes.c_int, "the Mip-Splatting 3D filter"),
    "stp_mip_activations_forward": ([ctypes.c_int] + [ctypes.c_void_p] * 6, ctypes.c_int, "the Mip-Splatting 3D filter"),
    "stp_mip_activations_backward": ([ctypes.c_int] + [ctypes.c_void_p] * 8, ctypes.c_int, "the Mip-Splatting 3D filter"),
    "stp_knn_scratch_bytes": ([ctypes.c_int], ctypes.c_size_t, "the nearest-neighbour kernels"),
    "stp_knn_mean_dist2": ([ctypes.c_int] + [ctypes.c_void_p] * 2 + [ctypes.c_size_t] + [ctypes.c_void_p] * 2, ctypes.c_int, "the nearest-neighbour kernels"),
    "stp_spatial_order_scratch_bytes": ([ctypes.c_int], ctypes.c_size_t, "the spatial order kernels"),
    "stp_spatial_order": ([ctypes.c_int] + [ctypes.c_void_p] * 2 + [ctypes.c_size_t] + [ctypes.c_void_p] * 3, ctypes.c_int, "the spatial order kernels"),
    "stp_gather_rows": ([ctypes.c_int] * 2 + [ctypes.c_void_p, ctypes.c_int] + [ctypes.c_void_p] * 2, ctypes.c_int, "the spatial order kernels"),
    "stp_densify_stats": ([ctypes.c_int] + [ctypes.c_void_p] * 4 + [ctypes.c_int, ctypes.c_void_p, ctypes.c_int, ctypes.c_void_p], ctypes.c_int, "the densification kernels"),
    "stp_densify_plan": ([ctypes.c_int] + [ctypes.c_void_p] * 8, ctypes.c_int, "the densification kernels"),
    "stp_densify_scratch_bytes": ([ctypes.c_int], ctypes.c_size_t, "the densification kernels"),
    "stp_densify_scan": ([ctypes.c_int] + [ctypes.c_void_p] * 2 + [ctypes.c_size_t] + [ctypes.c_void_p] * 3, ctypes.c_int, "the densification kernels"),
    "stp_densify_apply": ([ctypes.c_int] + [ctypes.c_void_p] * 3 + [ctypes.c_int] + [ctypes.c_void_p] * 2 + [ctypes.c_float, ctypes.c_int, ctypes.c_void_p],
                          ctypes.c_int, "the densification kernels"),
    "stp_photometric_workspace_floats": ([ctypes.c_int] * 3, ctypes.c_size_t, "the photometric loss"),
    "stp_photometric_forward": ([ctypes.c_int] * 3 + [ctypes.c_void_p] * 6, ctypes.c_int, "the photometric loss"),
    "stp_photometric_backward": ([ctypes.c_int] * 3 + [ctypes.c_void_p] * 6, ctypes.c_int, "the photometric loss"),
    "stp_training_loss_workspace_floats": ([ctypes.c_int] * 4, ctypes.c_size_t, "the training loss"),
    "stp_training_loss_forward": ([ctypes.c_int] * 3 + [ctypes.c_void_p] * 7, ctypes.c_int, "the training loss"),
    "stp_training_loss_backward": ([ctypes.c_int] * 3 + [ctypes.c_void_p] * 10, ctypes.c_int, "the training loss"),
}
_SYMBOL_FEATURE = {name: entry[2] for name, entry in _OPTIONAL_SYMBOLS.items()}


def _require(name: str):
    L = _load()
    if not hasattr(L, name):
        raise RuntimeError(f"{library_path()} does not export {name} (a library built before {_OPTIONAL_SYMBOLS[name][2]}): rebuild it")
    return getattr(L, name)


def camera_grad_workspace_bytes(P: int) -> int:
    return int(_require("stp_camera_grad_workspace_bytes")(int(P)))


def library_path() -> str:
    p = _lib_override or os.environ.get("STP_RASTER_LIB", os.path.join(_HERE, _LIB_NAME))
    return os.path.join(_HERE, "libstp_raster_fma.so") if p == "fma" else p


def use_library(path=None) -> None:
    global _lib, _host, _lib_override
    if path in ("fma", "default"):
        path = os.path.join(_HERE, "libstp_raster_fma.so" if path == "fma" else _LIB_NAME)
    _lib, _host, _lib_override = None, None, path


def _load():
    global _lib
    if _lib is not None:
        return _lib
    path = library_path()
    if not os.path.exists(path):
        raise ImportError(
            f"{path} not found: build it with `make -C stopthepop-rasterization_amd/csrc` "
            f"(or python -c 'import __graft_entry__ as g; g.build()'). There is no CPU fallback.")
    L = ctypes.CDLL(path)
    vp, ci, cf = ctypes.c_void_p, ctypes.c_int, ctypes.c_float
    L.stp_last_error.restype = ctypes.c_char_p
    L.stp_abi_version.restype = ci
    for name in ("stp_geometry_buffer_size", "stp_binning_buffer_size", "stp_image_buffer_size"):
        getattr(L, name).restype = ctypes.c_size_t
    L.stp_geometry_buffer_size.argtypes = [ci, ctypes.POINTER(StpSettings)]
    L.stp_binning_buffer_size.argtypes = [ci]
    L.stp_image_buffer_size.argtypes = [ci, ci]
    L.stp_blend_log_bytes.argtypes = [ci, ci]
    L.stp_blend_log_bytes.restype = ctypes.c_size_t
    szp = ctypes.POINTER(ctypes.c_size_t)
    L.stp_geometry_layout.argtypes = [ci, ctypes.POINTER(StpSettings), ctypes.c_char_p, szp, szp]
    L.stp_binning_layout.argtypes = [ci, ctypes.c_char_p, szp, szp]
    L.stp_image_layout.argtypes = [ci, ci, ctypes.c_char_p, szp, szp]
    L.stp_timing_enable.argtypes = [ci]
    L.stp_timing_enable.restype = None
    L.stp_timing_read.argtypes = [ctypes.POINTER(ctypes.c_float)]
    L.stp_timing_read.restype = ci
    L.stp_hbm_probe.argtypes = [ci, ctypes.c_void_p, ctypes.c_void_p, ctypes.c_size_t, ci, ctypes.c_void_p]
    L.stp_hbm_probe.restype = ci
    L.stp_timing_history.argtypes = [ctypes.POINTER(ctypes.c_float), ci]
    L.stp_timing_history.restype = ci
    L.stp_timing_history_host.argtypes = [ctypes.POINTER(ctypes.c_float), ci]
    L.stp_timing_history_host.restype = ci
    L.stp_timing_text.argtypes = [ctypes.c_char_p, ctypes.c_size_t]
    L.stp_timing_text.restype = ctypes.c_size_t
    L.stp_binning_layout_count.argtypes = [vp, ci]
    L.stp_binning_layout_count.restype = ci
    L.stp_forget_buffer.argtypes = [vp]
    L.stp_forget_buffer.restype = None
    for name in _OPTIONAL_SYMBOLS:
        if hasattr(L, name):
            fn = getattr(L, name)
            fn.argtypes, fn.restype = _OPTIONAL_SYMBOLS[name][:2]
    if L.stp_abi_version() != 7:
        raise ImportError("libstp_raster.so ABI version mismatch")
    _lib = L
    return L


def _native():
    global _host
    if _host is not None:
        return _host
    _load()
    try:
        from . import _stp_host
    except ImportError as ex:
        raise ImportError(f"the native host binding diff_gaussian_rasterization._stp_host is missing ({ex}): build it with "
                          f"`python stopthepop-rasterization_amd/csrc/host/build_host.py` (or python -c 'import __graft_entry__ as g; "
                          f"g.build()').  There is no pure-Python fallback.") from ex
    _stp_host.load_library(library_path())
    global _atexit_registered
    if not _atexit_registered:
        import atexit
        atexit.register(lambda: _stp_host.clear_scratch_pool(-1))
        _atexit_registered = True
    _host = _stp_host
    return _host


_atexit_registered = False


def settings_from_dict(d: dict, tile_rows=None) -> StpSettings:
    ss, cs = d["sort_settings"], d["culling_settings"]
    q = ss["queue_sizes"]
    s = StpSettings()
    s.sort_mode = int(ss["sort_mode"])
    s.sort_order = int(ss["sort_order"])
    s.queue_tile_4x4 = int(q["tile_4x4"])
    s.queue_tile_2x2 = int(q["tile_2x2"])
    s.queue_per_pixel = int(q["per_pixel"])
    s.rect_bounding = int(bool(cs["rect_bounding"]))
    s.tight_opacity_bounding = int(bool(cs["tight_opacity_bounding"]))
    s.tile_based_culling = int(bool(cs["tile_based_culling"]))
    s.hierarchical_4x4_culling = int(bool(cs["hierarchical_4x4_culling"]))
    s.load_balancing = int(bool(d["load_balancing"]))
    s.proper_ewa_scaling = int(bool(d["proper_ewa_scaling"]))
    tr = tile_rows if tile_rows is not None else d.get("_tile_rows")
    if tr is not None:
        s.tile_y0, s.tile_y1 = int(tr[0]), int(tr[1])
    if _records_log(d):
        s.record_blend_log = 1
    return s


_BACKWARD_MODES = ("replay", "resort", "auto")
_backward_mode = os.environ.get("STP_BACKWARD", "replay")
if _backward_mode not in _BACKWARD_MODES:
    raise ImportError(f"STP_BACKWARD={_backward_mode!r}: expected one of {_BACKWARD_MODES}")
_log_budget_bytes = int(float(os.environ.get("STP_LOG_BUDGET_GB", "16")) * (1 << 30))
_log_live = {}


def set_backward_mode(mode: str, log_budget_bytes=None) -> None:
    global _backward_mode, _log_budget_bytes
    if mode not in _BACKWARD_MODES:
        raise ValueError(f"backward mode {mode!r}: expected one of {_BACKWARD_MODES}")
    _backward_mode = mode
    if log_budget_bytes is not None:
        _log_budget_bytes = int(log_budget_bytes)


def backward_mode() -> str:
    return _backward_mode


def blend_log_bytes(width: int, height: int, tile_rows=None, depth=None) -> int:
    L = _load()
    y0, y1 = (0, 0) if tile_rows is None else (int(tile_rows[0]), int(tile_rows[1]))
    if depth is not None:
        L.stp_blend_log_bytes_depth.argtypes = [ctypes.c_int] * 5
        L.stp_blend_log_bytes_depth.restype = ctypes.c_size_t
        return int(L.stp_blend_log_bytes_depth(int(width), int(height), y0, y1, int(depth)))
    if tile_rows is None:
        return int(L.stp_blend_log_bytes(int(width), int(height)))
    L.stp_blend_log_bytes_rows.argtypes = [ctypes.c_int] * 4
    L.stp_blend_log_bytes_rows.restype = ctypes.c_size_t
    return int(L.stp_blend_log_bytes_rows(int(width), int(height), y0, y1))


class LogLease:

    def __init__(self, index: int, nbytes: int):
        self.index, self.nbytes = index, int(nbytes)
        _log_live[index] = _log_live.get(index, 0) + self.nbytes

    def resize(self, nbytes: int) -> None:
        if self.nbytes:
            _log_live[self.index] = _log_live.get(self.index, 0) - self.nbytes + int(nbytes)
            self.nbytes = int(nbytes)

    def release(self) -> None:
        if self.nbytes:
            _log_live[self.index] = _log_live.get(self.index, 0) - self.nbytes
            self.nbytes = 0

    __del__ = release


def live_log_bytes(device=None) -> int:
    return _log_live.get(_device_index(device), 0)


def decide_recording(mode, device, width: int, height: int, tile_rows=None) -> bool:
    mode = mode or _backward_mode
    if mode not in _BACKWARD_MODES:
        raise ValueError(f"backward mode {mode!r}: expected one of {_BACKWARD_MODES}")
    if mode != "auto":
        return mode == "replay"
    idx = _device_index(device)
    need = blend_log_bytes(width, height, tile_rows, depth=0)
    pooled = list(_native().pooled_sizes(idx))
    reuse = any(need <= n for n in pooled)
    return _log_live.get(idx, 0) + sum(pooled) + (0 if reuse else need) <= _log_budget_bytes


def _on_device(device):
    import contextlib
    return torch.cuda.device(_device_index(device)) if torch.cuda.is_available() else contextlib.nullcontext()


def _device_index(device) -> int:
    if device is None:
        return torch.cuda.current_device()
    if isinstance(device, int):
        return device
    d = torch.device(device)
    return torch.cuda.current_device() if d.index is None else d.index


def _raise_last(rc: int):
    msg = _load().stp_last_error()
    raise RuntimeError((msg.decode() if msg else "") or f"libstp_raster error {rc}")


def clear_scratch_pool(device=None) -> int:
    return int(_native().clear_scratch_pool(-1 if device is None else _device_index(device)))


def set_scratch_pool_limit(max_buffers: int = 4, max_bytes=None) -> None:
    _native().set_scratch_pool_limit(int(max_buffers), -1 if max_bytes is None else int(max_bytes))


def scratch_generation(buf: torch.Tensor) -> int:
    return int(_native().scratch_generation(buf))


def check_scratch(buf: torch.Tensor, generation: int) -> None:
    _native().check_scratch(buf, int(generation))


def set_forward_split(tile_row: int, event) -> None:
    _native().set_forward_split(int(tile_row), 0 if event is None else int(event.cuda_event))


def release_scratch(buf: torch.Tensor) -> None:
    _native().release_scratch(buf)


def _records_log(d: dict) -> bool:
    return bool(d.get("_record_blend_log")) and d.get("_backward_mode", _backward_mode) != "resort"


def rasterize_gaussians(background, means3D, colors, opacity, scales, rotations, scale_modifier, cov3D_precomp,
                        viewmatrix, projmatrix, inv_viewprojmatrix, tan_fovx, tan_fovy, image_height, image_width,
                        sh, degree, campos, prefiltered, settings_dict, render_depth, debug, alpha=False, invdepth=False,
                        raw=0, dc=None) -> Tuple[int, torch.Tensor, torch.Tensor, torch.Tensor, torch.Tensor, torch.Tensor]:
    if means3D.dim() != 2 or means3D.size(1) != 3:
        raise RuntimeError("means3D must have dimensions (num_points, 3)")
    if alpha or _per_pixel_background(background, image_height, image_width):
        _require("stp_set_forward_background")
    if invdepth:
        _require("stp_set_forward_invdepth")
        if render_depth:
            raise RuntimeError("the inverse-depth output (_invdepth) is not available with render_depth (the debug depth visualisation)")
    if dc is not None:
        _require("stp_set_forward_split_sh")
    if raw:
        _require("stp_set_forward_raw_params")
    out = (_host or _native()).rasterize_gaussians(
        background, means3D, colors, opacity, scales, rotations, scale_modifier, cov3D_precomp, viewmatrix, projmatrix,
        inv_viewprojmatrix, tan_fovx, tan_fovy, int(image_height), int(image_width), sh, int(degree), campos, bool(prefiltered),
        settings_dict, bool(render_depth), bool(debug), _records_log(settings_dict), bool(alpha), bool(invdepth), dc, int(raw))
    return tuple(out[:6]) + ((out[6],) if alpha else ()) + ((out[7],) if invdepth else ())


def _per_pixel_background(background, height, width) -> bool:
    return isinstance(background, torch.Tensor) and tuple(background.shape) == (3, int(height), int(width))


def rasterize_gaussians_backward(background, means3D, radii, opacities, colors, scales, rotations, scale_modifier,
                                 cov3D_precomp, viewmatrix, projmatrix, inv_viewprojmatrix, tan_fovx, tan_fovy,
                                 pixel_colors, dL_dout_color, sh, degree, campos, geomBuffer, R, binningBuffer,
                                 imageBuffer, settings_dict, debug, phases=3, partial=None, chunk=None, outputs=None,
                                 camera_grads=False, absgrad=False, blend_stats=False, dL_dalpha=None, bg_grad=False,
                                 dL_dinvdepth=None, invdepth=None, raw=0, dc=None):
    if chunk is not None:
        k, K = int(chunk[0]), int(chunk[1])
        if not (0 <= k < K <= 255) or (int(phases) & 1):
            raise ValueError("chunk = (k, K) with 0 <= k < K <= 255, per-Gaussian half only")
        phases = int(phases) | (K << 8) | (k << 16)
    if camera_grads:
        _require("stp_set_backward_camera_grads")
    if absgrad:
        _require("stp_set_backward_absgrad")
    if blend_stats:
        _require("stp_set_backward_blend_stats")
    if dL_dinvdepth is not None:
        _require("stp_set_backward_invdepth")
    if dc is not None:
        _require("stp_set_backward_split_sh")
    if raw:
        _require("stp_set_backward_raw_params")
    if dL_dalpha is not None or bg_grad or _per_pixel_background(background, dL_dout_color.shape[-2], dL_dout_color.shape[-1]):
        _require("stp_set_backward_background")
    out = (_host or _native()).rasterize_gaussians_backward(
        background, means3D, radii, opacities, colors, scales, rotations, scale_modifier, cov3D_precomp, viewmatrix, projmatrix,
        inv_viewprojmatrix, tan_fovx, tan_fovy, pixel_colors, dL_dout_color, sh, int(degree), campos, geomBuffer, int(R), binningBuffer,
        imageBuffer, settings_dict, bool(debug), _records_log(settings_dict), int(phases), partial, None if outputs is None else list(outputs),
        bool(camera_grads), bool(absgrad), bool(blend_stats), dL_dalpha, bool(bg_grad), dL_dinvdepth, invdepth, dc, int(raw))
    return out[0] if (int(phases) & 3) == 1 and not bg_grad else tuple(out)


def mark_visible(means3D, viewmatrix, projmatrix) -> torch.Tensor:
    return (_host or _native()).mark_visible(means3D, viewmatrix, projmatrix)


def sparse_adam(params, grads, exp_avgs, exp_avg_sqs, visible, lrs, epss, beta1, beta2, N) -> int:
    _require("stp_sparse_adam")
    return int((_host or _native()).sparse_adam(list(params), list(grads), list(exp_avgs), list(exp_avg_sqs), visible, [float(x) for x in lrs],
                                                [float(x) for x in epss], float(beta1), float(beta2), int(N)))


def adamUpdate(param, grad, exp_avg, exp_avg_sq, visible, lr, b1, b2, eps, N, M) -> None:
    if int(N) * int(M) != param.numel():
        raise RuntimeError(f"adamUpdate: param has {param.numel()} elements, N * M = {int(N) * int(M)}")
    sparse_adam([param], [grad], [exp_avg], [exp_avg_sq], visible, [lr], [eps], b1, b2, N)


DENSE_ADAM_REG_KINDS = {None: 0, "sigmoid": 1, "exp": 2}


def dense_adam_coefficients(lr, beta1, beta2, eps, step, reg_weight=0.0, numel=1):
    beta1, beta2, step = float(beta1), float(beta2), float(step)
    return (beta1, 1.0 - beta1, beta2, 1.0 - beta2, float(lr) / (1.0 - beta1 ** step), (1.0 - beta2 ** step) ** 0.5, float(eps),
            float(reg_weight) / max(int(numel), 1))


def dense_adam(params, grads, exp_avgs, exp_avg_sqs, coefs, reg_kinds) -> int:
    _require("stp_dense_adam")
    flat = [float(x) for c in coefs for x in c]
    return int((_host or _native()).dense_adam(list(params), list(grads), list(exp_avgs), list(exp_avg_sqs), flat, [int(k) for k in reg_kinds]))


RELOCATION_N_MAX = 51


def compute_relocation(opacity_old, scale_old, N, binoms=None, n_max=RELOCATION_N_MAX):
    _require("stp_mcmc_relocation")
    return tuple((_host or _native()).compute_relocation(opacity_old, scale_old, N, binoms, int(n_max)))


def mcmc_add_noise(xyz, scales, rotations, opacities, noise, noise_scale, k, x0, raw) -> int:
    _require("stp_mcmc_add_noise")
    return int((_host or _native()).mcmc_add_noise(xyz, scales, rotations, opacities, noise, float(noise_scale), float(k), float(x0), bool(raw)))


class StpMcmcTensor(ctypes.Structure):
    _fields_ = [(name, ctypes.c_void_p) for name in ("param", "exp_avg", "exp_avg_sq", "param_out", "exp_avg_out", "exp_avg_sq_out")] + \
               [("row", ctypes.c_int32), ("role", ctypes.c_int32)]


StpDensifyTensor = StpMcmcTensor

MCMC_ROLES = {"plain": 0, "opacity": 1, "scaling": 2}
MCMC_SAMPLE_TILE = 2048
MCMC_RELOCATE_MAX_P = 1 << 28


def mcmc_relocate_scratch_bytes(P: int) -> int:
    return int(_require("stp_mcmc_relocate_scratch_bytes")(int(P)))


def mcmc_sample(opacity, uniforms, rule, min_opacity, raw, want_weights):
    _require("stp_mcmc_sample")
    src, count, weights = (_host or _native()).mcmc_sample(opacity, uniforms, int(rule), float(min_opacity), bool(raw), bool(want_weights))
    return src, count, (weights if want_weights else None)


def mcmc_relocate_apply(src, count, tensors, roles, exp_avgs, exp_avg_sqs, min_opacity, raw, reset_dead_moments) -> int:
    _require("stp_mcmc_relocate_apply")
    return int((_host or _native()).mcmc_relocate_apply(src, count, list(tensors), [int(r) for r in roles], list(exp_avgs), list(exp_avg_sqs), float(min_opacity),
                                                        bool(raw), bool(reset_dead_moments)))


def mcmc_add_apply(src, count, tensors, roles, exp_avgs, exp_avg_sqs, min_opacity, raw):
    _require("stp_mcmc_add_apply")
    out = (_host or _native()).mcmc_add_apply(src, count, list(tensors), [int(r) for r in roles], list(exp_avgs), list(exp_avg_sqs), float(min_opacity), bool(raw))
    return list(out[0]), list(out[1]), list(out[2])


def activate_params(scaling=None, rotation=None, opacity=None):
    if scaling is None and rotation is None and opacity is None:
        return None, None, None
    _require("stp_activate_params")
    out = (_host or _native()).activate_params(scaling, rotation, opacity)
    return tuple(o if given is not None else None for o, given in zip(out, (scaling, rotation, opacity)))


def compute_3d_filter(xyz, world_view_transforms, intrinsics):
    _require("stp_mip_filter_3d")
    return (_host or _native()).compute_3d_filter(xyz, world_view_transforms, intrinsics)


def mip_activations(scaling, opacity, filter_3d):
    _require("stp_mip_activations_forward")
    return tuple((_host or _native()).mip_activations(scaling, opacity, filter_3d))


def mip_activations_backward(scaling, opacity, filter_3d, grad_scales, grad_opacities):
    _require("stp_mip_activations_backward")
    return tuple((_host or _native()).mip_activations_backward(scaling, opacity, filter_3d, grad_scales, grad_opacities))


KNN_BOX = 256


def knn_scratch_bytes(P: int) -> int:
    return int(_require("stp_knn_scratch_bytes")(int(P)))


def knn_mean_dist2(points):
    _require("stp_knn_mean_dist2")
    return (_host or _native()).knn_mean_dist2(points)


def spatial_order_scratch_bytes(P: int) -> int:
    return int(_require("stp_spatial_order_scratch_bytes")(int(P)))


def spatial_order(xyz, return_codes=False):
    _require("stp_spatial_order")
    _require("stp_spatial_order_scratch_bytes")
    order, codes = (_host or _native()).spatial_order(xyz, bool(return_codes))
    return order, (codes if return_codes else None)


class StpGatherTensor(ctypes.Structure):
    _fields_ = [(name, ctypes.c_void_p) for name in ("param", "exp_avg", "exp_avg_sq", "param_out", "exp_avg_out", "exp_avg_sq_out")] + \
               [("row", ctypes.c_int32), ("role", ctypes.c_int32)]


def gather_rows(index, tensors, exp_avgs, exp_avg_sqs):
    _require("stp_gather_rows")
    out = (_host or _native()).gather_rows(index, list(tensors), list(exp_avgs), list(exp_avg_sqs))
    return list(out[0]), list(out[1]), list(out[2])


class StpDensifyRule(ctypes.Structure):
    _fields_ = [(name, ctypes.c_float) for name in ("grad_threshold", "split_size", "min_opacity", "max_screen_size", "max_world_size", "split_shrink")] + \
               [("raw", ctypes.c_int32), ("prune_big", ctypes.c_int32)]


DENSIFY_ROLES = {"plain": 0, "xyz": 1, "scaling": 2, "rotation": 3}


def densify_stats(xyz_gradient_accum, denom, max_radii2D, grad2d, radii) -> int:
    _require("stp_densify_stats")
    return int((_host or _native()).densify_stats(xyz_gradient_accum, denom, max_radii2D, grad2d, radii))


def densify_plan(xyz_gradient_accum, denom, scaling, opacity, max_radii2D, rule, raw, prune_big):
    _require("stp_densify_plan")
    return (_host or _native()).densify_plan(xyz_gradient_accum, denom, scaling, opacity, max_radii2D, [float(x) for x in rule], bool(raw), bool(prune_big))


def densify_scan(plan):
    _require("stp_densify_scan")
    offsets, nK, nC, nS = (_host or _native()).densify_scan(plan)
    return offsets, (int(nK), int(nC), int(nS))


def densify_apply(plan, offsets, counts, tensors, roles, exp_avgs, exp_avg_sqs, noise, split_shrink, raw):
    _require("stp_densify_apply")
    out = (_host or _native()).densify_apply(plan, offsets, [int(c) for c in counts], list(tensors), [int(r) for r in roles], list(exp_avgs),
                                             list(exp_avg_sqs), noise, float(split_shrink), bool(raw))
    return list(out[0]), list(out[1]), list(out[2])


def photometric_forward(image, target, want_maps):
    for name in ("stp_photometric_workspace_floats", "stp_photometric_forward", "stp_photometric_backward"):
        _require(name)
    out2, maps = (_host or _native()).photometric_forward(image, target, bool(want_maps))
    return out2, (maps if want_maps else None)


def photometric_backward(image, target, maps, grad_out2):
    _require("stp_photometric_backward")
    return (_host or _native()).photometric_backward(image, target, maps, grad_out2)


class StpTrainingLoss(ctypes.Structure):
    _fields_ = [(n, ctypes.c_void_p) for n in ("exposure", "alpha_mask", "invdepth", "mono_invdepth", "depth_mask")] + \
               [(n, ctypes.c_int32) for n in ("clamp", "exposure_batched", "alpha_mask_batched", "channels", "depth_planes")]


_TRAINING_LOSS_SYMBOLS = ("stp_training_loss_workspace_floats", "stp_training_loss_forward", "stp_training_loss_backward")


def training_loss_forward(image, target, exposure, clamp, alpha_mask, invdepth, mono_invdepth, depth_mask, want_maps):
    for name in _TRAINING_LOSS_SYMBOLS:
        _require(name)
    out3, maps = (_host or _native()).training_loss_forward(image, target, exposure, bool(clamp), alpha_mask, invdepth, mono_invdepth, depth_mask, bool(want_maps))
    return out3, (maps if want_maps else None)


def training_loss_backward(image, target, exposure, clamp, alpha_mask, invdepth, mono_invdepth, depth_mask, maps, grad_out3, want_exposure, want_invdepth):
    _require("stp_training_loss_backward")
    g_image, g_exposure, g_invdepth = (_host or _native()).training_loss_backward(image, target, exposure, bool(clamp), alpha_mask, invdepth, mono_invdepth, depth_mask,
                                                                                  maps, grad_out3, bool(want_exposure), bool(want_invdepth))
    return g_image, (g_exposure if want_exposure else None), (g_invdepth if want_invdepth else None)


_GEOM_TYPES = {"depths": torch.float32, "clamped": torch.uint8, "radii": torch.int32, "rects2D": torch.float32,
               "means2D": torch.float32, "cov3D": torch.float32, "cov3D_inv": torch.float32,
               "conic_opacity": torch.float32, "rgb": torch.float32, "tiles_touched": torch.int32,
               "point_offsets": torch.int32, "invz": torch.float32,
               "sh_stash": torch.float32}
_BIN_TYPES = {"point_list": torch.int32, "point_list_unsorted": torch.int32, "keys": torch.int64, "keys_unsorted": torch.int64}
_IMG_TYPES = {"final_T": torch.float32, "n_contrib": torch.int32, "ranges": torch.int32, "tile_flags": torch.int32,
              "blend_log": torch.int16}


def timing_text(device=None) -> str:
    buf = ctypes.create_string_buffer(512)
    with _on_device(device):
        _load().stp_timing_text(buf, 512)
    return buf.value.decode()


def _view(buf: torch.Tensor, off: int, count: int, dtype) -> torch.Tensor:
    nbytes = count * torch.empty((), dtype=dtype).element_size()
    return buf[off:off + nbytes].view(dtype)


def has_sh_stash(geomBuffer, P, settings_dict) -> bool:
    if geomBuffer.numel() < 48:
        return False
    w = geomBuffer[32:44].view(torch.int32).cpu().tolist()
    return (w[0] & 0xFFFFFFFF) == 0x53505453 and (w[1] & 0xFFFFFFFF) == int(P) and (w[2] & 0xFFFFFFFF) == (~int(P) & 0xFFFFFFFF)


def geometry_array(geomBuffer, P, settings_dict, name):
    s = settings_from_dict(settings_dict)
    off, cnt = ctypes.c_size_t(), ctypes.c_size_t()
    if _load().stp_geometry_layout(int(P), ctypes.byref(s), name.encode(), ctypes.byref(off), ctypes.byref(cnt)) != 0:
        raise KeyError(name)
    return _view(geomBuffer, off.value, cnt.value, _GEOM_TYPES[name])


def binning_array(binningBuffer, R, name):
    off, cnt = ctypes.c_size_t(), ctypes.c_size_t()
    L = _load()
    if binningBuffer.is_cuda:
        _native().forget_unless_same_storage(binningBuffer)
    lay = int(L.stp_binning_layout_count(ctypes.c_void_p(binningBuffer.data_ptr()), int(R))) if int(R) > 0 else 0
    if lay < 0:
        _raise_last(lay)
    if L.stp_binning_layout(lay, name.encode(), ctypes.byref(off), ctypes.byref(cnt)) != 0:
        raise KeyError(name)
    n = cnt.value // lay * int(R) if lay > 0 else cnt.value
    return _view(binningBuffer, off.value, n, _BIN_TYPES[name])


def image_array(imgBuffer, W, H, name, tile_rows=None):
    off, cnt = ctypes.c_size_t(), ctypes.c_size_t()
    L = _load()
    L.stp_image_layout_depth.argtypes = [ctypes.c_int] * 5 + [ctypes.c_char_p, ctypes.POINTER(ctypes.c_size_t), ctypes.POINTER(ctypes.c_size_t)]
    y0, y1 = (0, 0) if tile_rows is None else (int(tile_rows[0]), int(tile_rows[1]))
    depth = blend_log_depth(imgBuffer) if name == "blend_log" else 0
    if L.stp_image_layout_depth(int(W), int(H), y0, y1, depth, name.encode(), ctypes.byref(off), ctypes.byref(cnt)) != 0:
        raise KeyError(name)
    return _view(imgBuffer, off.value, cnt.value, _IMG_TYPES[name])


def blend_log_depth(imgBuffer) -> int:
    L = _load()
    L.stp_blend_log_depth.argtypes = [ctypes.c_void_p]
    L.stp_blend_log_depth.restype = ctypes.c_int
    if imgBuffer.is_cuda:
        _native().forget_unless_same_storage(imgBuffer)
    d = int(L.stp_blend_log_depth(ctypes.c_void_p(imgBuffer.data_ptr())))
    if d < 0:
        _raise_last(d)
    return d


def set_run_ahead(mode) -> int:
    L = _load()
    L.stp_set_run_ahead.argtypes = [ctypes.c_int]
    L.stp_set_run_ahead.restype = None
    L.stp_get_run_ahead.restype = ctypes.c_int
    prev = int(L.stp_get_run_ahead())
    L.stp_set_run_ahead(int(mode))
    return prev


def reset_size_guesses() -> None:
    L = _load()
    L.stp_reset_size_guesses.restype = None
    L.stp_reset_size_guesses()


def timing_enable(flag: bool) -> None:
    _load().stp_timing_enable(int(bool(flag)))


def hbm_probe(kind: str, dst, src, blocks: int = 4096, nontemporal: bool = False) -> None:
    import torch
    t = src if src is not None else dst
    k = {"read": 0, "write": 1, "copy": 2}[kind] + (4 if nontemporal else 0)
    with _on_device(t.device):
        rc = _load().stp_hbm_probe(k, None if dst is None else dst.data_ptr(), None if src is None else src.data_ptr(),
                                   t.numel() * t.element_size(), int(blocks), torch.cuda.current_stream(t.device).cuda_stream)
    if rc < 0:
        raise RuntimeError(f"stp_hbm_probe failed ({rc})")


def timing_history(device=None, capacity=1024, host=False):
    arr = (ctypes.c_float * (6 * capacity))()
    with _on_device(device):
        n = (_load().stp_timing_history_host if host else _load().stp_timing_history)(arr, capacity)
    if n < 0:
        _raise_last(n)
    names = ("Preprocess", "Duplicate", "Sort", "Render", "BwdRender", "BwdPreprocess")
    return [{nm: float(arr[6 * k + i]) for i, nm in enumerate(names) if arr[6 * k + i] >= 0.0} for k in range(n)]


def timing_read(device=None):
    arr = (ctypes.c_float * 6)()
    with _on_device(device):
        rc = _load().stp_timing_read(arr)
    if rc < 0:
        _raise_last(rc)
    names = ("Preprocess", "Duplicate", "Sort", "Render", "BwdRender", "BwdPreprocess")
    return {n: float(v) for n, v in zip(names, arr)}
```

Baseline: 462.1.

## Compute onesweep digit histograms in preprocess and skip the sort histogram pass

Preprocess now counts the 8-bit tile-key digits of each Gaussian's touched tiles into a shared-memory histogram and flushes it atomically to global memory. The block-prefix mailbox kernel scans those counts into per-place digit offsets, padding the top digit for the speculative capacity. The onesweep sort then takes these offsets and skips its own histogram and scan kernels, which saves a full read pass over the unsorted keys. In exchange preprocess does extra shared atomics and runs at 512 threads per block, and the speculative padding and overflow handling add correctness risk.

```diff
diff --git a/stopthepop-rasterization_amd/csrc/stp_binning.hip b/stopthepop-rasterization_amd/csrc/stp_binning.hip
--- a/stopthepop-rasterization_amd/csrc/stp_binning.hip
+++ b/stopthepop-rasterization_amd/csrc/stp_binning.hip
@@ -59,6 +59,7 @@
 constexpr unsigned OS_HIST_ITEMS = OS.histogram.block_size * OS.histogram.items_per_thread;
 constexpr unsigned OS_SORT_ITEMS = OS.sort.block_size * OS.sort.items_per_thread;
 constexpr unsigned OS_MAX_PLACES = 4;
+static_assert(OS_MAX_PLACES == (unsigned)SORT_HIST_PLACES && OS_RADIX == (unsigned)SORT_HIST_RADIX, "stp_internal.h: SortHist is laid out for these passes");
 using OsBlockId = rpd::block_id_wrapper<unsigned int, true>;
 
 struct OsLayout {
@@ -146,13 +147,26 @@
 #endif
 }
 
+SortHist sort_hist_for(const FrameParams& f, uint32_t* block)
+{
+    SortHist h{};
+    const Switches& sw = switches();
+    if (!STP_OWN_ONESWEEP || block == nullptr || !sw.tile_local_sort || sw.atomic_bin || !sw.two_level_scan || sw.tile_sort == Switches::TILE_SORT_ROCPRIM || sw.sort_hist_keys) return h;
+    const int bit = (int)higher_msb((uint32_t)(f.gx * f.gy));
+    h.places = (bit + 7) / 8;
+    if (h.places < 1 || h.places > SORT_HIST_PLACES) return SortHist{};
+    h.last_bits = bit - 8 * (h.places - 1);
+    h.counts = block; h.offsets = block + SORT_HIST_WORDS;
+    return h;
+}
+
 hipError_t launch_scan(const FrameParams& f, const GeometryState& g, hipStream_t st)
 {
     size_t bytes = g.scan_temp_bytes;
     return rocprim::inclusive_scan(g.scan_temp, bytes, g.tiles_touched, g.point_offsets, (size_t)f.P, rocprim::plus<uint32_t>(), st);
 }
 
-hipError_t launch_sort(const FrameParams& f, const BinningState& b, int R, bool tile_bits_only, bool zeroed, hipStream_t st)
+hipError_t launch_sort(const FrameParams& f, const BinningState& b, int R, bool tile_bits_only, bool zeroed, const uint32_t* upstream_offsets, hipStream_t st)
 {
     if (R <= 0) return hipSuccess;
     const uint32_t bit = higher_msb((uint32_t)(f.gx * f.gy));
@@ -166,7 +180,9 @@
     const unsigned begin_bit = 32u, end_bit = 32u + bit;
     const unsigned places = (bit + OS.radix_bits_per_place - 1) / OS.radix_bits_per_place;
     const uint32_t size = (uint32_t)R;
-    {
+    static_assert(OS.radix_bits_per_place == 8, "sort_hist_for and preprocess_kernel count eight-bit digits");
+    uint32_t* const offsets = upstream_offsets ? const_cast<uint32_t*>(upstream_offsets) : L.offsets;
+    if (!upstream_offsets) {
         const uint32_t blocks = (size + OS_HIST_ITEMS - 1) / OS_HIST_ITEMS, full_blocks = size % OS_HIST_ITEMS == 0 ? blocks : blocks - 1;
         hipLaunchKernelGGL(os_histograms_kernel, dim3(blocks), dim3(OS.histogram.block_size), 0, st, b.keys_unsorted, L.offsets, size, full_blocks, begin_bit, end_bit);
         hipLaunchKernelGGL(os_scan_histograms_kernel, dim3(places), dim3(OS.histogram.block_size), 0, st, L.offsets);
@@ -179,7 +195,7 @@
         uint64_t* kout = to_output ? b.keys : L.keys_tmp;
         uint32_t* vout = to_output ? b.point_list : L.values_tmp;
         const unsigned radix_bits = end_bit - pbit < OS.radix_bits_per_place ? end_bit - pbit : OS.radix_bits_per_place;
-        hipLaunchKernelGGL(os_iteration_kernel, dim3(blocks), dim3(OS.sort.block_size), 0, st, kin, kout, vin, vout, size, L.offsets + place * OS_RADIX, L.offsets_tmp,
+        hipLaunchKernelGGL(os_iteration_kernel, dim3(blocks), dim3(OS.sort.block_size), 0, st, kin, kout, vin, vout, size, offsets + place * OS_RADIX, L.offsets_tmp,
                            L.lookback + (size_t)place * OS_RADIX * blocks, pbit, radix_bits, full_blocks, OsBlockId::create(L.block_ids + place));
         from_input = false;
         to_output = !to_output;
diff --git a/stopthepop-rasterization_amd/csrc/stp_buffers.hip b/stopthepop-rasterization_amd/csrc/stp_buffers.hip
--- a/stopthepop-rasterization_amd/csrc/stp_buffers.hip
+++ b/stopthepop-rasterization_amd/csrc/stp_buffers.hip
@@ -7,7 +7,7 @@
 
 namespace stp {
 
-GeometryState carve_geometry(char* base, size_t P, bool with_inv, size_t* total, NamedOffset* names, int* n_names, float** sh_stash)
+GeometryState carve_geometry(char* base, size_t P, bool with_inv, size_t* total, NamedOffset* names, int* n_names, float** sh_stash, uint32_t** sort_hist)
 {
     Carver c(base);
     GeometryState g{};
@@ -33,6 +33,10 @@
     g.scan_temp = c.take<char>(g.scan_temp_bytes);
     g.invz = c.take<float>(P, &off); note("invz", off, P);
     {
+        uint32_t* const hist = c.take<uint32_t>(2 * (size_t)SORT_HIST_WORDS, &off); note("sort_offsets", off + sizeof(uint32_t) * SORT_HIST_WORDS, SORT_HIST_WORDS);
+        if (sort_hist) *sort_hist = hist;
+    }
+    {
         const Carver before_stash = c;
         float* const stash = c.take<float>(9 * P, &off); note("sh_stash", off, 9 * P);
         if (sh_stash) *sh_stash = stash;
diff --git a/stopthepop-rasterization_amd/csrc/stp_forward.hip b/stopthepop-rasterization_amd/csrc/stp_forward.hip
--- a/stopthepop-rasterization_amd/csrc/stp_forward.hip
+++ b/stopthepop-rasterization_amd/csrc/stp_forward.hip
@@ -111,6 +111,7 @@
     bool colour_started = true;
     char* bin_ptr = nullptr; size_t bin_have = 0;
     uint32_t cap = 0; bool ahead = false, run_ahead = false;
+    uint32_t* sort_hist_block = nullptr; SortHist hist{};
     int* radii; float* const out_color;
     struct Split { const ForwardSplit s; hipStream_t st; bool recorded; ~Split() { if (s.armed && !recorded) (void)hipEventRecord(s.event, st); } } split;
     SideJoin colours;
@@ -118,19 +119,19 @@
     ForwardCall(hipStream_t stream, int debug_, const ForwardSplit& split_, int* radii_, float* out_color_)
         : st(stream), debug(debug_), radii(radii_), out_color(out_color_), split{split_, stream, false}, colours{nullptr, stream, false} {}
     int carve_geometry_and_image(stp_alloc_fn geometry_alloc, void* geometry_user, stp_alloc_fn image_alloc, void* image_user, bool with_inv, bool with_stash);
-    int launch_up_to_mailbox(); int colour_on_side();
+    void choose_capacity(); int launch_up_to_mailbox(); int colour_on_side();
     int request_binning(stp_alloc_fn binning_alloc, void* binning_user);
     int wait_mailbox(); int read_mailbox(int* R_out, bool* wild_out);
-    int binning_and_render(const GeometryState& gd, const BinningState& b, int L, uint32_t dup_cap);
+    int binning_and_render(const GeometryState& gd, const BinningState& b, int L, uint32_t dup_cap, bool upstream_offsets);
 };
 
 int ForwardCall::carve_geometry_and_image(stp_alloc_fn geometry_alloc, void* geometry_user, stp_alloc_fn image_alloc, void* image_user, bool with_inv, bool with_stash)
 {
     size_t geom_bytes = 0;
-    carve_geometry(nullptr, (size_t)f.P, with_inv, &geom_bytes, nullptr, nullptr, with_stash ? &sh_stash : nullptr);
+    carve_geometry(nullptr, (size_t)f.P, with_inv, &geom_bytes, nullptr, nullptr, with_stash ? &sh_stash : nullptr, nullptr);
     char* geom_ptr = (char*)geometry_alloc(geometry_user, geom_bytes);
     if (!geom_ptr) return fail(STP_ERR_ALLOC, "geometry allocator returned NULL");
-    g = carve_geometry(geom_ptr, (size_t)f.P, with_inv, nullptr, nullptr, nullptr, with_stash ? &sh_stash : nullptr);
+    g = carve_geometry(geom_ptr, (size_t)f.P, with_inv, nullptr, nullptr, nullptr, with_stash ? &sh_stash : nullptr, &sort_hist_block);
     geom_base = geom_ptr;
     if (!radii) radii = g.internal_radii;
 
@@ -159,14 +160,15 @@
     const bool atomic_bin = switches().atomic_bin, two_level_scan = switches().two_level_scan;
     timer_begin_forward();
     timer_mark(0, st);
-    STP_TRY(launch_frame_init(g, img, f.gx * f.ty0, f.gx * (f.ty1 - f.ty0), with_log, atomic_bin, st), "frame init launch");
-    STP_TRY(launch_preprocess(f, g, radii, atomic_bin ? img.tile_counts : nullptr, st), "preprocess launch");
+    hist = sort_hist_for(f, sort_hist_block);
+    STP_TRY(launch_frame_init(g, img, f.gx * f.ty0, f.gx * (f.ty1 - f.ty0), with_log, atomic_bin, sort_hist_block, st), "frame init launch");
+    STP_TRY(launch_preprocess(f, g, radii, atomic_bin ? img.tile_counts : nullptr, hist, st), "preprocess launch");
     STP_DEBUG_SYNC("preprocess");
     if (!two_level_scan) STP_TRY(launch_scan(f, g, st), "inclusive scan");
     STP_DEBUG_SYNC("scan");
     if (atomic_bin) STP_TRY(launch_tile_scan(f, img, st), "tile scan");
 
-    if (two_level_scan) STP_TRY(launch_block_prefix_mailbox(f, g, mb.dev, mb.ticket, log_need_word, st), "workgroup prefixes + mailbox launch");
+    if (two_level_scan) STP_TRY(launch_block_prefix_mailbox(f, g, mb.dev, mb.ticket, log_need_word, hist, ahead ? cap : 0u, st), "workgroup prefixes + mailbox launch");
     else STP_TRY(launch_mailbox(g.point_offsets + (f.P - 1), g.status + 1, mb.dev, mb.ticket, log_need_word, st), "mailbox launch");
     STP_TRY(hipEventRecord(mb.ev, st), "record mailbox event");
     side = side_stream(mb.device);
@@ -189,7 +191,7 @@
     return 0;
 }
 
-int ForwardCall::request_binning(stp_alloc_fn binning_alloc, void* binning_user)
+void ForwardCall::choose_capacity()
 {
     const Switches& sw = switches();
     const int run_ahead_mode = g_run_ahead.load(std::memory_order_relaxed);
@@ -197,7 +199,10 @@
     const uint32_t guess = (sw.speculative_binning && gslot->key.load(std::memory_order_acquire) == gkey) ? gslot->R.load(std::memory_order_relaxed) : 0u;
     ahead = run_ahead && guess > 0 && (run_ahead_mode == 1 || guess < RUN_AHEAD_AUTO_MAX) && sw.two_level_scan && !sw.atomic_bin && !debug;
     cap = guess + guess / 8 + (ahead ? 1024u : 0u);
-    if (guess > 0) {
+}
+int ForwardCall::request_binning(stp_alloc_fn binning_alloc, void* binning_user)
+{
+    if (cap > 0) {
         carve_binning(nullptr, (size_t)cap, &bin_have);
         bin_ptr = (char*)binning_alloc(binning_user, bin_have);
         if (!bin_ptr) return fail(STP_ERR_ALLOC, "binning allocator returned NULL");
@@ -244,7 +249,7 @@
     return 0;
 }
 
-int ForwardCall::binning_and_render(const GeometryState& gd, const BinningState& b, int L, uint32_t dup_cap)
+int ForwardCall::binning_and_render(const GeometryState& gd, const BinningState& b, int L, uint32_t dup_cap, bool upstream_offsets)
 {
     const bool atomic_bin = switches().atomic_bin, tile_local_sort = switches().tile_local_sort;
     uint32_t* zero_ptr = nullptr; size_t zero_words = 0;
@@ -260,7 +265,7 @@
     if (atomic_bin) {
         STP_TRY(launch_bin_pad(b, img, L, st), "pad entries");
     } else {
-        STP_TRY(launch_sort(f, b, L, tile_local_sort, zero_words != 0, st), "radix sort");
+        STP_TRY(launch_sort(f, b, L, tile_local_sort, zero_words != 0, upstream_offsets ? hist.offsets : nullptr, st), "radix sort");
         STP_DEBUG_SYNC("sort");
         STP_TRY(launch_ranges(f, b, img, L, st), "tile ranges");
         STP_DEBUG_SYNC("ranges");
@@ -372,6 +377,7 @@
     f.fused_gather = sw.fused_gather && sw.tile_local_sort && !sw.atomic_bin && f.s.sort_mode == MODE_HIER && f.s.debug_visualization != STP_DEBUG_DEPTH ? 1 : 0;
     if (!sw.two_level_scan) { c.g.block_sums = nullptr; c.g.block_prefix = nullptr; }
 
+    c.choose_capacity();
     if (int rc = c.launch_up_to_mailbox()) return rc;
     if (int rc = c.request_binning(binning_alloc, binning_user)) return rc;
 
@@ -383,7 +389,7 @@
         f.wild_cov = 0;
         timer_mark(1, st);
         const BinningState b = carve_binning(c.bin_ptr, (size_t)c.cap, nullptr);
-        if (int rc = c.binning_and_render(g_dup, b, (int)c.cap, c.cap)) return rc;
+        if (int rc = c.binning_and_render(g_dup, b, (int)c.cap, c.cap, true)) return rc;
         if (int rc = c.read_mailbox(&R, &wild)) return rc;
         if ((uint32_t)R <= c.cap && !wild) {
             remember_stash(c.geom_base, with_stash, R);
@@ -392,7 +398,7 @@
             return R;
         }
         g_dup.block_prefix = nullptr; g_dup.block_sums = nullptr;
-        STP_TRY(launch_frame_init(c.g, c.img, f.gx * f.ty0, f.gx * (f.ty1 - f.ty0), c.with_log, sw.atomic_bin, st), "frame init launch");
+        STP_TRY(launch_frame_init(c.g, c.img, f.gx * f.ty0, f.gx * (f.ty1 - f.ty0), c.with_log, sw.atomic_bin, nullptr, st), "frame init launch");
         STP_TRY(launch_stash_mark(f, c.g, c.sh_stash, st), "stash mark launch");
     } else {
         if (int rc = c.read_mailbox(&R, &wild)) return rc;
@@ -407,7 +413,7 @@
         if (!c.bin_ptr) return fail(STP_ERR_ALLOC, "binning allocator returned NULL");
     }
     const BinningState b = carve_binning(c.bin_ptr, (size_t)R, nullptr);
-    if (int rc = c.binning_and_render(g_dup, b, R, 0xFFFFFFFFu)) return rc;
+    if (int rc = c.binning_and_render(g_dup, b, R, 0xFFFFFFFFu, !c.ahead)) return rc;
     remember_stash(c.geom_base, with_stash, R);
     if (c.bin_ptr) remember_layout(c.bin_ptr, (uint32_t)R, R);
     remember_log_depth(c.img_ptr, (uint32_t)c.log_depth, R);
diff --git a/stopthepop-rasterization_amd/csrc/stp_internal.h b/stopthepop-rasterization_amd/csrc/stp_internal.h
--- a/stopthepop-rasterization_amd/csrc/stp_internal.h
+++ b/stopthepop-rasterization_amd/csrc/stp_internal.h
@@ -74,6 +74,13 @@
 };
 constexpr int STP_STASH_WORD = 8;
 constexpr uint32_t STP_HEADER_MAGIC_STASH = 0x53505453u;
+constexpr int SORT_HIST_PLACES = 4, SORT_HIST_RADIX = 256, SORT_HIST_WORDS = SORT_HIST_PLACES * SORT_HIST_RADIX;
+struct SortHist {
+    uint32_t* counts = nullptr;
+    uint32_t* offsets = nullptr;
+    int places = 0;
+    int last_bits = 0;
+};
 
 struct ImageState {
     float* final_T;
@@ -107,7 +114,7 @@
 constexpr uint32_t STP_HEADER_MAGIC_BINNING = 0x42505453u, STP_HEADER_MAGIC_IMAGE = 0x49505453u;
 struct NamedOffset { const char* name; size_t offset; size_t count; };
 
-GeometryState carve_geometry(char* base, size_t P, bool with_inv, size_t* total, NamedOffset* names = nullptr, int* n_names = nullptr, float** sh_stash = nullptr);
+GeometryState carve_geometry(char* base, size_t P, bool with_inv, size_t* total, NamedOffset* names = nullptr, int* n_names = nullptr, float** sh_stash = nullptr, uint32_t** sort_hist = nullptr);
 ImageState carve_image(char* base, int W, int H, int ty0, int ty1, int log_depth , size_t* total, NamedOffset* names = nullptr, int* n_names = nullptr);
 BinningState carve_binning(char* base, size_t R, size_t* total, NamedOffset* names = nullptr, int* n_names = nullptr);
 void clamp_tile_rows(int height, int& y0, int& y1);
@@ -212,8 +219,9 @@
 ForwardRequests take_forward_requests();
 int check_raw_params(int mask, const float* opacities, const float* scales, const float* rotations);
 
-hipError_t launch_preprocess(const FrameParams& f, const GeometryState& g, int* radii, uint32_t* tile_counts, hipStream_t st);
-hipError_t launch_frame_init(const GeometryState& g, const ImageState& img, int tile0, int n_tiles, bool with_log, bool tile_counters, hipStream_t st);
+hipError_t launch_preprocess(const FrameParams& f, const GeometryState& g, int* radii, uint32_t* tile_counts, const SortHist& hist, hipStream_t st);
+hipError_t launch_frame_init(const GeometryState& g, const ImageState& img, int tile0, int n_tiles, bool with_log, bool tile_counters, uint32_t* sort_counts, hipStream_t st);
+SortHist sort_hist_for(const FrameParams& f, uint32_t* block);
 hipError_t launch_scan(const FrameParams& f, const GeometryState& g, hipStream_t st);
 bool tile_order_enabled();
 inline bool tile_order_used(const FrameParams& f) { return tile_order_enabled() && f.gx * (f.ty1 - f.ty0) > 1024; }
@@ -223,11 +231,11 @@
 hipError_t launch_sh_color(const FrameParams& f, const GeometryState& g, const int* radii, float* sh_stash, hipStream_t st);
 hipError_t launch_stash_mark(const FrameParams& f, const GeometryState& g, float* sh_stash, hipStream_t st);
 hipError_t launch_mailbox(const uint32_t* last_offset, const uint32_t* status, uint32_t* mailbox_dev, uint32_t ticket, uint32_t* log_need, hipStream_t st);
-hipError_t launch_block_prefix_mailbox(const FrameParams& f, const GeometryState& g, uint32_t* mailbox_dev, uint32_t ticket, uint32_t* log_need, hipStream_t st);
+hipError_t launch_block_prefix_mailbox(const FrameParams& f, const GeometryState& g, uint32_t* mailbox_dev, uint32_t ticket, uint32_t* log_need, const SortHist& hist, uint32_t cap, hipStream_t st);
 hipError_t launch_duplicate(const FrameParams& f, const GeometryState& g, const int* radii, const BinningState& b, uint32_t* tile_cursor, uint32_t cap, uint32_t header_cap, uint32_t* zero_ptr, size_t zero_words, hipStream_t st);
 hipError_t launch_tile_scan(const FrameParams& f, const ImageState& img, hipStream_t st);
 hipError_t launch_bin_pad(const BinningState& b, const ImageState& img, int R, hipStream_t st);
-hipError_t launch_sort(const FrameParams& f, const BinningState& b, int R, bool tile_bits_only, bool zeroed, hipStream_t st);
+hipError_t launch_sort(const FrameParams& f, const BinningState& b, int R, bool tile_bits_only, bool zeroed, const uint32_t* upstream_offsets, hipStream_t st);
 void sort_zero_region(const BinningState& b, size_t R, uint32_t tiles, uint32_t** ptr, size_t* words);
 hipError_t launch_tile_sort_gather(const FrameParams& f, const GeometryState& g, const BinningState& b, const ImageState& img, int R, bool unordered, hipStream_t st);
 hipError_t launch_ranges(const FrameParams& f, const BinningState& b, const ImageState& img, int R, hipStream_t st);
diff --git a/stopthepop-rasterization_amd/csrc/stp_preprocess.hip b/stopthepop-rasterization_amd/csrc/stp_preprocess.hip
--- a/stopthepop-rasterization_amd/csrc/stp_preprocess.hip
+++ b/stopthepop-rasterization_amd/csrc/stp_preprocess.hip
@@ -25,6 +25,9 @@
     int* radii;
     GeometryState g;
     uint32_t* tile_counts;
+    uint32_t* hist;
+    int hist_places;
+    int n_blocks;
 };
 
 __device__ __forceinline__ void sh_to_rgb(int idx, int deg, float3 mean, float3 cam, const float* __restrict__ sh,
@@ -195,10 +198,16 @@
     return true;
 }
 
-__global__ void __launch_bounds__(256) preprocess_kernel(const PreArgs a)
+__device__ __forceinline__ void count_tile_digits(uint32_t* __restrict__ s_hist, int places, uint32_t tile)
+{
+    for (int p = 0; p < places; p++) atomicAdd(&s_hist[p * SORT_HIST_RADIX + (int)((tile >> (8 * p)) & 255u)], 1u);
+}
+
+template <bool COUNT>
+__device__ __forceinline__ void preprocess_block(const PreArgs& a, const int block, const int t, uint32_t* __restrict__ s_hist, uint32_t* __restrict__ s_wave_total)
 {
 #pragma clang fp contract(off)
-    const int idx = blockIdx.x * blockDim.x + threadIdx.x;
+    const int idx = block * 256 + t;
     PreStageA o{};
     bool alive = false;
     if (idx < a.P) {
@@ -212,7 +221,8 @@
     int full_count = 1;
     const bool tbc = a.tile_based_culling != 0;
     const int rect_tiles = (o.fx1 - o.fx0) * (o.fy1 - o.fy0);
-    const bool coop = alive && tbc && a.tile_counts == nullptr && rect_tiles > COOP_TILES;
+    constexpr bool count_digits = COUNT;
+    const bool coop = alive && (tbc || count_digits) && a.tile_counts == nullptr && rect_tiles > COOP_TILES;
     if (alive && tbc && !coop) {
         tile_count = 0;
         full_count = 0;
@@ -227,10 +237,14 @@
                 const int mine = (y >= y0 && y < y1) ? hit : 0;
                 tile_count += mine;
                 if (mine && a.tile_counts) atomicAdd(&a.tile_counts[y * a.gx + x], 1u);
+                if (mine && count_digits) count_tile_digits(s_hist, a.hist_places, (uint32_t)(y * a.gx + x));
             }
-    } else if (alive && !tbc && a.tile_counts) {
+    } else if (alive && !tbc && !coop && (a.tile_counts || count_digits)) {
         for (int y = y0; y < y1; y++)
-            for (int x = x0; x < x1; x++) atomicAdd(&a.tile_counts[y * a.gx + x], 1u);
+            for (int x = x0; x < x1; x++) {
+                if (a.tile_counts) atomicAdd(&a.tile_counts[y * a.gx + x], 1u);
+                if (count_digits) count_tile_digits(s_hist, a.hist_places, (uint32_t)(y * a.gx + x));
+            }
     }
     {
         const int lane = wave_lane();
@@ -253,10 +267,12 @@
                     const float2 tmin = make_float2((float)(x * TILE), (float)(y * TILE));
                     const float2 tmax = make_float2((float)((x + 1) * TILE - 1), (float)((y + 1) * TILE - 1));
                     float2 mp;
-                    hit = max_contrib_power_rect(co, m2, tmin, tmax, (float)(TILE - 1), (float)(TILE - 1), mp) <= thr;
+                    hit = !tbc || max_contrib_power_rect(co, m2, tmin, tmax, (float)(TILE - 1), (float)(TILE - 1), mp) <= thr;
                 }
+                const bool in_window = hit && y >= wy0 && y < wy1;
                 full += (int)__popcll(__ballot(hit));
-                mine += (int)__popcll(__ballot(hit && y >= wy0 && y < wy1));
+                mine += (int)__popcll(__ballot(in_window));
+                if (in_window && count_digits) count_tile_digits(s_hist, a.hist_places, (uint32_t)(y * a.gx + x));
             }
             if (lane == src) { full_count = full; tile_count = mine; }
         }
@@ -272,8 +288,14 @@
     const float3 cam = make_float3(a.cam[0], a.cam[1], a.cam[2]);
 
     if (a.g.cov3D_inv != nullptr) {
-        const float3 sc = o.sc;
-        const float4 q = o.q;
+        float3 sc = o.sc;
+        float4 q = o.q;
+        if constexpr (COUNT) {
+            sc = make_float3(a.scales[3 * (size_t)idx], a.scales[3 * (size_t)idx + 1], a.scales[3 * (size_t)idx + 2]);
+            q = reinterpret_cast<const float4*>(a.rotations)[idx];
+            if (a.raw & RAW_SCALE) sc = make_float3(activate_scale(sc.x), activate_scale(sc.y), activate_scale(sc.z));
+            if (a.raw & RAW_ROTATION) q = activate_rotation(q, nullptr);
+        }
         const Mat3 S = mat_diag(1.f / (a.scale_modifier * fmaxf(1e-3f, sc.x)), 1.f / (a.scale_modifier * fmaxf(1e-3f, sc.y)),
                                 1.f / (a.scale_modifier * fmaxf(1e-3f, sc.z)));
         const Mat3 Mm = mat_mul(S, quat_to_mat(q));
@@ -314,8 +336,7 @@
     }
 
     if (a.g.block_sums != nullptr) {
-        __shared__ uint32_t s_wave_total[4];
-        const int lane = wave_lane(), wave = (int)(threadIdx.x >> 6);
+        const int lane = wave_lane(), wave = t >> 6;
         uint32_t v = my_entries;
 #pragma unroll
         for (int d = 1; d < 64; d <<= 1) {
@@ -326,7 +347,24 @@
         __syncthreads();
         for (int k = 0; k < wave; k++) v += s_wave_total[k];
         if (idx < a.P) a.g.point_offsets[idx] = v;
-        if (threadIdx.x == 255) a.g.block_sums[blockIdx.x] = v;
+        if (t == 255 && block < a.n_blocks) a.g.block_sums[block] = v;
+    }
+}
+
+template <int BLOCKS, bool COUNT>
+__global__ void __launch_bounds__(256 * BLOCKS) preprocess_kernel(const PreArgs a)
+{
+    __shared__ uint32_t s_hist[SORT_HIST_WORDS];
+    __shared__ uint32_t s_wave_total[4 * BLOCKS];
+    const int tid = (int)threadIdx.x, sub = tid >> 8;
+    const int bins = COUNT ? a.hist_places * SORT_HIST_RADIX : 0;
+    for (int i = tid; i < bins; i += 256 * BLOCKS) s_hist[i] = 0u;
+    if (bins) __syncthreads();
+    preprocess_block<COUNT>(a, (int)blockIdx.x * BLOCKS + sub, tid & 255, s_hist, s_wave_total + 4 * sub);
+    if (bins) __syncthreads();
+    for (int i = tid; i < bins; i += 256 * BLOCKS) {
+        const uint32_t c = s_hist[i];
+        if (c) atomicAdd(&a.hist[i], c);
     }
 }
 
@@ -640,7 +678,10 @@
 
 }
 
-hipError_t launch_preprocess(const FrameParams& f, const GeometryState& g, int* radii, uint32_t* tile_counts, hipStream_t st)
+#ifndef STP_PRE_BLOCKS
+#define STP_PRE_BLOCKS 2
+#endif
+hipError_t launch_preprocess(const FrameParams& f, const GeometryState& g, int* radii, uint32_t* tile_counts, const SortHist& hist, hipStream_t st)
 {
     PreArgs a;
     a.P = f.P; a.D = f.D; a.M = f.M; a.W = f.W; a.H = f.H; a.gx = f.gx; a.gy = f.gy; a.ty0 = f.ty0; a.ty1 = f.ty1;
@@ -652,7 +693,10 @@
     a.cov3D_precomp = f.cov3D_precomp; a.colors_precomp = f.colors_precomp; a.view = f.viewmatrix; a.proj = f.projmatrix; a.cam = f.cam_pos;
     a.radii = radii; a.g = g; a.tile_counts = tile_counts;
     if (f.out_invdepth == nullptr) a.g.invz = nullptr;
-    hipLaunchKernelGGL(preprocess_kernel, dim3((f.P + 255) / 256), dim3(256), 0, st, a);
+    a.hist = hist.counts; a.hist_places = hist.places;
+    a.n_blocks = (f.P + 255) / 256;
+    if (hist.counts) hipLaunchKernelGGL((preprocess_kernel<STP_PRE_BLOCKS, true>), dim3((a.n_blocks + STP_PRE_BLOCKS - 1) / STP_PRE_BLOCKS), dim3(256 * STP_PRE_BLOCKS), 0, st, a);
+    else hipLaunchKernelGGL((preprocess_kernel<1, false>), dim3(a.n_blocks), dim3(256), 0, st, a);
     return hipGetLastError();
 }
 
@@ -716,10 +760,13 @@
 
 __global__ void __launch_bounds__(1024) block_prefix_mailbox_kernel(const uint32_t* __restrict__ block_sums, uint32_t* __restrict__ block_prefix, int n_blocks,
                                                                      const uint32_t* __restrict__ status, volatile uint32_t* mailbox, uint32_t ticket,
-                                                                     uint32_t* log_need)
+                                                                     uint32_t* log_need, const SortHist hist, uint32_t cap)
 {
     __shared__ uint32_t s_wave_total[16];
+    __shared__ uint32_t s_digit_total[16];
     const int tid = (int)threadIdx.x, lane = tid & 63, wave = tid >> 6;
+    const bool digit_mine = hist.counts != nullptr && (tid >> 8) < hist.places;
+    uint32_t digit_count = digit_mine ? hist.counts[tid] : 0u;
     const int per = (n_blocks + 1023) / 1024, i0 = min(tid * per, n_blocks), i1 = min(i0 + per, n_blocks);
     uint32_t mine = 0u;
     for (int i = i0; i < i1; i++) mine += block_sums[i];
@@ -742,11 +789,28 @@
         mailbox[2] = ticket;
         __threadfence_system();
     }
-}
-
-hipError_t launch_block_prefix_mailbox(const FrameParams& f, const GeometryState& g, uint32_t* mailbox_dev, uint32_t ticket, uint32_t* log_need, hipStream_t st)
-{
-    hipLaunchKernelGGL(block_prefix_mailbox_kernel, dim3(1), dim3(1024), 0, st, g.block_sums, g.block_prefix, (f.P + 255) / 256, g.status, mailbox_dev, ticket, log_need);
+    if (hist.counts == nullptr) return;
+    uint32_t total = 0u;
+    for (int k = 0; k < 16; k++) total += s_wave_total[k];
+    const bool overflow = cap != 0u && total > cap;
+    const int place = tid >> 8, pad_digit = (1 << (place == hist.places - 1 ? hist.last_bits : 8)) - 1;
+    if (digit_mine && cap != 0u && !overflow && (tid & 255) == pad_digit) digit_count += cap - total;
+    uint32_t d = digit_count;
+#pragma unroll
+    for (int s = 1; s < 64; s <<= 1) {
+        const uint32_t t = (uint32_t)__shfl_up((int)d, s);
+        if (lane >= s) d += t;
+    }
+    if (lane == 63) s_digit_total[wave] = d;
+    __syncthreads();
+    for (int k = wave & ~3; k < wave; k++) d += s_digit_total[k];
+    if (digit_mine) hist.offsets[tid] = overflow ? 0u : d - digit_count;
+}
+
+hipError_t launch_block_prefix_mailbox(const FrameParams& f, const GeometryState& g, uint32_t* mailbox_dev, uint32_t ticket, uint32_t* log_need, const SortHist& hist, uint32_t cap, hipStream_t st)
+{
+    hipLaunchKernelGGL(block_prefix_mailbox_kernel, dim3(1), dim3(1024), 0, st, g.block_sums, g.block_prefix, (f.P + 255) / 256, g.status, mailbox_dev, ticket, log_need, hist,
+                       hist.counts ? cap : 0u);
     return hipGetLastError();
 }
 
@@ -758,9 +822,11 @@
 
 __global__ void __launch_bounds__(256) frame_init_kernel(uint32_t* __restrict__ status, uint2* __restrict__ ranges, uint32_t* __restrict__ tile_flags,
                                                           uint32_t flag_value, uint32_t* __restrict__ tile_counts, int tile0, int T,
-                                                          uint32_t* __restrict__ header, uint32_t log_depth)
+                                                          uint32_t* __restrict__ header, uint32_t log_depth, uint32_t* __restrict__ sort_counts)
 {
     const int i = blockIdx.x * blockDim.x + threadIdx.x;
+    if (sort_counts)
+        for (int j = i; j < 2 * SORT_HIST_WORDS; j += (int)(gridDim.x * blockDim.x)) sort_counts[j] = 0u;
     if (i < 64) status[i] = 0u;
     if (i == 0) { header[0] = STP_HEADER_MAGIC_IMAGE; header[1] = log_depth; header[2] = ~log_depth; header[3] = 0u; }
     if (i < T) {
@@ -770,11 +836,11 @@
     }
 }
 
-hipError_t launch_frame_init(const GeometryState& g, const ImageState& img, int tile0, int T, bool with_log, bool tile_counters, hipStream_t st)
+hipError_t launch_frame_init(const GeometryState& g, const ImageState& img, int tile0, int T, bool with_log, bool tile_counters, uint32_t* sort_counts, hipStream_t st)
 {
     const int n = T > 64 ? T : 64;
     hipLaunchKernelGGL(frame_init_kernel, dim3((n + 255) / 256), dim3(256), 0, st, g.status, img.ranges, img.tile_flags, with_log ? 0u : 0xFFFFFFFFu,
-                       tile_counters ? img.tile_counts : nullptr, tile0, T, img.header, (uint32_t)(with_log ? img.log_depth : 0));
+                       tile_counters ? img.tile_counts : nullptr, tile0, T, img.header, (uint32_t)(with_log ? img.log_depth : 0), sort_counts);
     return hipGetLastError();
 }
 
diff --git a/stopthepop-rasterization_amd/csrc/stp_switches.h b/stopthepop-rasterization_amd/csrc/stp_switches.h
--- a/stopthepop-rasterization_amd/csrc/stp_switches.h
+++ b/stopthepop-rasterization_amd/csrc/stp_switches.h
@@ -19,6 +19,7 @@
     bool tile_order;
     int gather_order;
     enum TileSort { TILE_SORT_AUTO, TILE_SORT_ROCPRIM, TILE_SORT_OWN } tile_sort;
+    bool sort_hist_keys;
     enum KBuffer { KBUFFER_RING, KBUFFER_TILE, KBUFFER_WAVE } kbuffer;
 };
 
@@ -43,6 +44,7 @@
         s.tile_order = !starts_with_0("STP_TILE_ORDER");
         s.gather_order = number("STP_GATHER_ORDER");
         s.tile_sort = is("STP_TILE_SORT", "rocprim") ? Switches::TILE_SORT_ROCPRIM : is("STP_TILE_SORT", "own") ? Switches::TILE_SORT_OWN : Switches::TILE_SORT_AUTO;
+        s.sort_hist_keys = is("STP_SORT_HIST", "keys");
         s.kbuffer = is("STP_KBUFFER", "tile") ? Switches::KBUFFER_TILE : is("STP_KBUFFER", "wave") ? Switches::KBUFFER_WAVE : Switches::KBUFFER_RING;
         return s;
     }();
diff --git a/stopthepop-rasterization_amd/diff_gaussian_rasterization/_C.py b/stopthepop-rasterization_amd/diff_gaussian_rasterization/_C.py
--- a/stopthepop-rasterization_amd/diff_gaussian_rasterization/_C.py
+++ b/stopthepop-rasterization_amd/diff_gaussian_rasterization/_C.py
@@ -578,6 +578,7 @@
                "means2D": torch.float32, "cov3D": torch.float32, "cov3D_inv": torch.float32,
                "conic_opacity": torch.float32, "rgb": torch.float32, "tiles_touched": torch.int32,
                "point_offsets": torch.int32, "invz": torch.float32,
+               "sort_offsets": torch.int32,
                "sh_stash": torch.float32}
 _BIN_TYPES = {"point_list": torch.int32, "point_list_unsorted": torch.int32, "keys": torch.int64, "keys_unsorted": torch.int64}
 _IMG_TYPES = {"final_T": torch.float32, "n_contrib": torch.int32, "ranges": torch.int32, "tile_flags": torch.int32,
```

Result: no change. 462.0 (-0.0%).
